# Angel3245/p2pfl

Hardware: AMD Instinct MI355X
Metric: train samples/s (aggregate over peers); wall-clock per FedAvg round in ms_per_step (higher is better)
Workload: dtype bf16; 1 GPU; model=MNIST-CNN (p2pfl CNN: conv5x5 32/64 + FC 3136-2048-10, 6.5M params), Adam 1e-3, global_batch=32, per_peer_round=2700 train + 300 val + 500 test samples, 1 epoch, parallelism=gossip-p2p

## Files before the change

### csrc/cnn.h

```cpp
#pragma once
#include <hip/hip_runtime.h>
#include <stdint.h>

namespace p2cnn {

constexpr int kImg = 28;
constexpr int kC1 = 32;
constexpr int kC2 = 64;
constexpr int kFeat = 3136;
constexpr int kHid = 2048;
constexpr int kCls = 10;
constexpr int kTaps = 25;
constexpr int kXcdSplits = 7;
bool xcd_align();

struct AdamCfg {
  float lr, beta1, beta2, eps, weight_decay;
};

struct Offsets {
  int64_t c1w, c1b, c2w, c2b, l1w, l1b, l2w, l2b;
};

void conv1_fwd(const uint8_t* x, const int64_t* idx, const float* params, Offsets off, uint16_t* p1, uint8_t* am1,
               uint16_t* p1s, int B, hipStream_t s);

void conv2_fwd(const uint16_t* p1, const uint16_t* w2r, const float* params, Offsets off, uint16_t* a1, uint8_t* am2,
               int B, hipStream_t s);

void conv12_fwd(const uint8_t* x, const int64_t* idx, const float* params, Offsets off, const uint16_t* w2r,
                uint16_t* p1, uint8_t* am1, uint16_t* p1s, uint16_t* a1, uint8_t* am2, int B, hipStream_t s);

void gemm_skinny(const uint16_t* A, const uint16_t* Bt, float* slabs, int mrows, int N, int K, int S, hipStream_t s);

void head(const float* slabs, int S, int mrows, const float* params, Offsets off, const int64_t* labels,
          const int64_t* idx, int B, int train, uint16_t* H, uint16_t* dH, float* dlogits, float* stats,
          const uint16_t* w2bf, hipStream_t s);

void fc1_wgrad_adam(const uint16_t* dH, const uint16_t* a1, int mrows, float* params, float* m, float* v,
                    float* gdump, uint16_t* w1bf, uint16_t* w1tbf, Offsets off, const int* adam_t, int t_off,
                    AdamCfg cfg, hipStream_t s);

void route_fc2(const uint16_t* dH, const uint16_t* w1t, const uint8_t* am2, int mrows, int B, uint16_t* dc2m,
               float* gb, const float* dlogits, const uint16_t* H, float* params, float* m, float* v, float* gdump,
               Offsets off, const int* adam_t, int t_off, AdamCfg cfg, bool with_fc2, hipStream_t s);

void route_fc2_rm(const uint16_t* dH, const uint16_t* w1, const uint8_t* am2, int mrows, int B, uint16_t* dc2m,
                  float* gb, const float* dlogits, const uint16_t* H, float* params, float* m, float* v,
                  float* gdump, Offsets off, const int* adam_t, int t_off, AdamCfg cfg, bool with_fc2,
                  float* ws, int* ctr, hipStream_t s);

void conv2_bwd(const uint16_t* dc2m, const uint16_t* p1s, const uint8_t* am1, const uint16_t* w2q, const uint8_t* x,
               const int64_t* idx, float* wslab1, float* wslab2, int B, hipStream_t s);

constexpr int kFc1Tiles = ((kFeat + 127) / 128) * (kHid / 32);
struct Fc1Args {
  const uint16_t* dH;
  const uint16_t* a1;
  int mrows;
  float* params;
  float* m;
  float* v;
  float* gdump;
  uint16_t* w1bf;
  uint16_t* w1tbf;
  Offsets off;
  const int* adam_t;
  int t_off;
  AdamCfg cfg;
};

int conv2_bwd_fc1(const uint16_t* dc2m, const uint16_t* p1s, const uint8_t* am1, const uint16_t* w2q, const uint8_t* x,
                  const int64_t* idx, float* wslab1, float* wslab2, int B, const Fc1Args& f, int n_tiles,
                  hipStream_t s);

void conv_adam(const float* wslab1, const float* wslab2, const float* gb, int B, float* params, float* m, float* v,
               float* gdump, uint16_t* w2r, uint16_t* w2q, Offsets off, const int* adam_t, int t_off, AdamCfg cfg,
               hipStream_t s);

struct FwdNext {
  const uint8_t* x;
  const int64_t* idx;
  uint16_t* p1;
  uint8_t* am1;
  uint16_t* p1s;
  uint16_t* a1;
  uint8_t* am2;
  int B;
  int* sync;
};
void fc1_conv_adam_fwd(const uint16_t* dH, const uint16_t* a1, int mrows, const float* wslab1, const float* wslab2,
                       const float* gb, int B, float* params, float* m, float* v, float* gdump, uint16_t* w1bf,
                       uint16_t* w1tbf, uint16_t* w2r, uint16_t* w2q, Offsets off, const int* adam_t, int t_off,
                       AdamCfg cfg, const float* dlogits, const uint16_t* H, uint16_t* w2bf, const FwdNext& f,
                       hipStream_t s);

void fc1_conv_adam(const uint16_t* dH, const uint16_t* a1, int mrows, const float* wslab1, const float* wslab2,
                   const float* gb, int B, float* params, float* m, float* v, float* gdump, uint16_t* w1bf,
                   uint16_t* w1tbf, uint16_t* w2r, uint16_t* w2q, Offsets off, const int* adam_t, int t_off,
                   AdamCfg cfg, const float* dlogits, const uint16_t* H, uint16_t* w2bf, int first_tile,
                   hipStream_t s);

void pack_shadows(const float* params, Offsets off, uint16_t* w2r, uint16_t* w2q, uint16_t* w1bf, uint16_t* w1tbf,
                  uint16_t* w2bf, hipStream_t s);

constexpr int kP1sPlane = 18 * 16;
constexpr int kP1s = 5 * kC1 * kP1sPlane;
constexpr int kDgTiles = 7;
constexpr int kSlab1 = kC1 * kTaps + kC1;
constexpr int kWgG = 2;
constexpr int kSlab2 = kTaps * kC2 * kC1;
__host__ __device__ inline int wgrad_groups(int B) { return (B + kWgG - 1) / kWgG; }

}
```

### csrc/cnn_bindings.cpp

```cpp
#include <torch/extension.h>
#include <c10/hip/HIPStream.h>
#include <c10/core/DeviceGuard.h>

#include "cnn.h"

namespace {

using p2cnn::AdamCfg;
using p2cnn::Offsets;

hipStream_t stream() { return c10::hip::getCurrentHIPStream().stream(); }

template <typename T>
T* ptr(const torch::Tensor& t, c10::ScalarType st, int64_t min_numel, const char* name, int align = 16) {
  TORCH_CHECK(t.defined() && t.is_cuda(), name, ": expected a GPU tensor");
  TORCH_CHECK(t.scalar_type() == st, name, ": wrong dtype ", t.scalar_type());
  TORCH_CHECK(t.is_contiguous(), name, ": must be contiguous");
  TORCH_CHECK(t.numel() >= min_numel, name, ": needs >= ", min_numel, " elements, got ", t.numel());
  TORCH_CHECK(reinterpret_cast<uintptr_t>(t.data_ptr()) % align == 0, name, ": must be ", align, "-byte aligned");
  return reinterpret_cast<T*>(t.data_ptr());
}
template <typename T>
T* optr(const c10::optional<torch::Tensor>& t, c10::ScalarType st, int64_t min_numel, const char* name,
        int align = 16) {
  if (!t.has_value() || !t->defined()) return nullptr;
  return ptr<T>(*t, st, min_numel, name, align);
}

Offsets offsets(const std::vector<int64_t>& o) {
  TORCH_CHECK(o.size() == 8, "offsets: expected 8 entries");
  for (auto v : o) TORCH_CHECK(v >= 0, "offsets: negative");
  return Offsets{o[0], o[1], o[2], o[3], o[4], o[5], o[6], o[7]};
}

int64_t params_end(const Offsets& o) {
  return std::max({o.c1w + 800, o.c1b + 32, o.c2w + 51200, o.c2b + 64, o.l1w + int64_t(2048) * 3136, o.l1b + 2048,
                   o.l2w + 20480, o.l2b + 10});
}

void check_batch(int B, int mrows) {
  TORCH_CHECK(mrows == 32 || mrows == 64 || mrows == 128, "mrows must be 32, 64 or 128");
  TORCH_CHECK(B >= 1 && B <= mrows, "batch ", B, " exceeds mrows ", mrows);
}

const int64_t* idx_ptr(const c10::optional<torch::Tensor>& idx, int B) {
  return optr<int64_t>(idx, torch::kInt64, B, "idx", 8);
}


void k_conv1_fwd(torch::Tensor x, c10::optional<torch::Tensor> idx, torch::Tensor params, std::vector<int64_t> off,
                 torch::Tensor p1, torch::Tensor am1, c10::optional<torch::Tensor> p1s, int64_t B) {
  const c10::DeviceGuard g(params.device());
  TORCH_CHECK(B >= 1 && B <= (p1s.has_value() && p1s->defined() ? 64 : 128), "bad batch");
  Offsets o = offsets(off);
  TORCH_CHECK(x.numel() % 784 == 0, "x must be [N,1,28,28] uint8");
  if (!idx.has_value()) TORCH_CHECK(x.numel() / 784 >= B, "x has fewer than B rows");
  p2cnn::conv1_fwd(ptr<uint8_t>(x, torch::kUInt8, 784, "x", 1), idx_ptr(idx, B),
                   ptr<float>(params, torch::kFloat32, params_end(o), "params"), o,
                   reinterpret_cast<uint16_t*>(ptr<at::BFloat16>(p1, torch::kBFloat16, B * 196 * 32, "p1")),
                   ptr<uint8_t>(am1, torch::kUInt8, B * 196 * 32, "am1"),
                   reinterpret_cast<uint16_t*>(optr<at::BFloat16>(p1s, torch::kBFloat16, B * p2cnn::kP1s, "p1s")),
                   int(B), stream());
}

void k_conv2_fwd(torch::Tensor p1, torch::Tensor w2r, torch::Tensor params, std::vector<int64_t> off,
                 torch::Tensor a1, torch::Tensor am2, int64_t B, int64_t mrows) {
  const c10::DeviceGuard g(params.device());
  check_batch(int(B), int(mrows));
  Offsets o = offsets(off);
  p2cnn::conv2_fwd(reinterpret_cast<uint16_t*>(ptr<at::BFloat16>(p1, torch::kBFloat16, B * 196 * 32, "p1")),
                   reinterpret_cast<uint16_t*>(ptr<at::BFloat16>(w2r, torch::kBFloat16, 51200, "w2r")),
                   ptr<float>(params, torch::kFloat32, params_end(o), "params"), o,
                   reinterpret_cast<uint16_t*>(ptr<at::BFloat16>(a1, torch::kBFloat16, mrows * 3136, "a1")),
                   ptr<uint8_t>(am2, torch::kUInt8, B * 3136, "am2"), int(B), stream());
}

void k_conv12_fwd(torch::Tensor x, c10::optional<torch::Tensor> idx, torch::Tensor params, std::vector<int64_t> off,
                  torch::Tensor w2r, c10::optional<torch::Tensor> p1, torch::Tensor am1, c10::optional<torch::Tensor> p1s,
                  torch::Tensor a1, torch::Tensor am2, int64_t B, int64_t mrows) {
  const c10::DeviceGuard g(params.device());
  check_batch(int(B), int(mrows));
  TORCH_CHECK(!(p1s.has_value() && p1s->defined()) || B <= 64, "conv12_fwd: training launches hold <= 64 images");
  Offsets o = offsets(off);
  TORCH_CHECK(x.numel() % 784 == 0, "x must be [N,1,28,28] uint8");
  if (!idx.has_value()) TORCH_CHECK(x.numel() / 784 >= B, "x has fewer than B rows");
  p2cnn::conv12_fwd(ptr<uint8_t>(x, torch::kUInt8, 784, "x", 1), idx_ptr(idx, int(B)),
                    ptr<float>(params, torch::kFloat32, params_end(o), "params"), o,
                    reinterpret_cast<uint16_t*>(ptr<at::BFloat16>(w2r, torch::kBFloat16, 51200, "w2r")),
                    reinterpret_cast<uint16_t*>(optr<at::BFloat16>(p1, torch::kBFloat16, B * 196 * 32, "p1")),
                    ptr<uint8_t>(am1, torch::kUInt8, B * 196 * 32, "am1"),
                    reinterpret_cast<uint16_t*>(optr<at::BFloat16>(p1s, torch::kBFloat16, B * p2cnn::kP1s, "p1s")),
                    reinterpret_cast<uint16_t*>(ptr<at::BFloat16>(a1, torch::kBFloat16, mrows * 3136, "a1")),
                    ptr<uint8_t>(am2, torch::kUInt8, B * 3136, "am2"), int(B), stream());
}

void k_gemm_skinny(torch::Tensor A, torch::Tensor Bt, torch::Tensor slabs, int64_t mrows, int64_t N, int64_t K,
                   int64_t S) {
  const c10::DeviceGuard g(A.device());
  TORCH_CHECK(N % 32 == 0 && K % 64 == 0 && S >= 1, "gemm_skinny: N%32, K%64 required");
  TORCH_CHECK(mrows == 32 || mrows == 64 || mrows == 128, "gemm_skinny: mrows must be 32, 64 or 128");
  p2cnn::gemm_skinny(reinterpret_cast<uint16_t*>(ptr<at::BFloat16>(A, torch::kBFloat16, mrows * K, "A")),
                     reinterpret_cast<uint16_t*>(ptr<at::BFloat16>(Bt, torch::kBFloat16, N * K, "Bt")),
                     ptr<float>(slabs, torch::kFloat32, S * mrows * N, "slabs"), int(mrows), int(N), int(K), int(S),
                     stream());
}

void k_head(torch::Tensor slabs, int64_t S, int64_t mrows, torch::Tensor params, std::vector<int64_t> off,
            torch::Tensor labels, c10::optional<torch::Tensor> idx, int64_t B, bool train, torch::Tensor H,
            torch::Tensor dH, torch::Tensor dlogits, torch::Tensor stats, c10::optional<torch::Tensor> w2bf) {
  const c10::DeviceGuard g(params.device());
  check_batch(int(B), int(mrows));
  Offsets o = offsets(off);
  if (!idx.has_value()) TORCH_CHECK(labels.numel() >= B, "labels has fewer than B rows");
  p2cnn::head(ptr<float>(slabs, torch::kFloat32, S * mrows * 2048, "slabs"), int(S), int(mrows),
              ptr<float>(params, torch::kFloat32, params_end(o), "params"), o,
              ptr<int64_t>(labels, torch::kInt64, 1, "labels", 8), idx_ptr(idx, B), int(B), train ? 1 : 0,
              reinterpret_cast<uint16_t*>(ptr<at::BFloat16>(H, torch::kBFloat16, mrows * 2048, "H")),
              reinterpret_cast<uint16_t*>(ptr<at::BFloat16>(dH, torch::kBFloat16, mrows * 2048, "dH")),
              ptr<float>(dlogits, torch::kFloat32, mrows * 10, "dlogits"), ptr<float>(stats, torch::kFloat32, 2, "stats", 4),
              reinterpret_cast<const uint16_t*>(optr<at::BFloat16>(w2bf, torch::kBFloat16, 10 * 2048, "w2bf")),
              stream());
}

AdamCfg cfg(double lr, double b1, double b2, double eps, double wd) {
  return AdamCfg{float(lr), float(b1), float(b2), float(eps), float(wd)};
}

void k_fc1_wgrad_adam(torch::Tensor dH, torch::Tensor a1, int64_t mrows, torch::Tensor params, torch::Tensor m,
                      torch::Tensor v, c10::optional<torch::Tensor> gdump, torch::Tensor w1bf, c10::optional<torch::Tensor> w1tbf,
                      std::vector<int64_t> off, torch::Tensor adam_t, int64_t t_off, double lr, double b1, double b2,
                      double eps, double wd) {
  const c10::DeviceGuard g(params.device());
  TORCH_CHECK(mrows == 32 || mrows == 64, "mrows must be 32 or 64");
  Offsets o = offsets(off);
  const int64_t n = params_end(o);
  p2cnn::fc1_wgrad_adam(reinterpret_cast<uint16_t*>(ptr<at::BFloat16>(dH, torch::kBFloat16, mrows * 2048, "dH")),
                        reinterpret_cast<uint16_t*>(ptr<at::BFloat16>(a1, torch::kBFloat16, mrows * 3136, "a1")),
                        int(mrows), ptr<float>(params, torch::kFloat32, n, "params"),
                        ptr<float>(m, torch::kFloat32, n, "m"), ptr<float>(v, torch::kFloat32, n, "v"),
                        optr<float>(gdump, torch::kFloat32, n, "gdump"),
                        reinterpret_cast<uint16_t*>(ptr<at::BFloat16>(w1bf, torch::kBFloat16, 2048 * 3136, "w1bf")),
                        reinterpret_cast<uint16_t*>(optr<at::BFloat16>(w1tbf, torch::kBFloat16, 2048 * 3136, "w1tbf")),
                        o, ptr<int>(adam_t, torch::kInt32, 1, "adam_t", 4), int(t_off), cfg(lr, b1, b2, eps, wd), stream());
}

void k_route_fc2(torch::Tensor dH, torch::Tensor w1, torch::Tensor am2, int64_t mrows, int64_t B,
                 torch::Tensor dc2m, torch::Tensor gb, torch::Tensor dlogits, torch::Tensor H, torch::Tensor params,
                 torch::Tensor m, torch::Tensor v, c10::optional<torch::Tensor> gdump, std::vector<int64_t> off,
                 torch::Tensor adam_t, int64_t t_off, double lr, double b1, double b2, double eps, double wd,
                 bool with_fc2, bool row_major, c10::optional<torch::Tensor> ws, c10::optional<torch::Tensor> ctr) {
  const c10::DeviceGuard g(dH.device());
  check_batch(int(B), int(mrows));
  TORCH_CHECK(mrows <= 64, "route_fc2: mrows must be 32 or 64");
  TORCH_CHECK(ws.has_value() == ctr.has_value(), "route_fc2: split-K needs both ws and ctr");
  TORCH_CHECK(!ws.has_value() || row_major, "route_fc2: split-K only on the row-major W1 kernel");
  Offsets o = offsets(off);
  const int64_t n = params_end(o);
  const auto dHp = reinterpret_cast<uint16_t*>(ptr<at::BFloat16>(dH, torch::kBFloat16, mrows * 2048, "dH"));
  const auto w1p = reinterpret_cast<uint16_t*>(ptr<at::BFloat16>(w1, torch::kBFloat16, 2048 * 3136, "w1"));
  const auto am2p = ptr<uint8_t>(am2, torch::kUInt8, B * 3136, "am2");
  const auto dc2p = reinterpret_cast<uint16_t*>(ptr<at::BFloat16>(dc2m, torch::kBFloat16, B * 64 * 224, "dc2m"));
  const auto gbp = ptr<float>(gb, torch::kFloat32, B * 3136, "gb");
  const auto dlp = ptr<float>(dlogits, torch::kFloat32, B * 10, "dlogits");
  const auto Hp = reinterpret_cast<uint16_t*>(ptr<at::BFloat16>(H, torch::kBFloat16, B * 2048, "H"));
  float* pp = ptr<float>(params, torch::kFloat32, n, "params");
  float* mp = ptr<float>(m, torch::kFloat32, n, "m");
  float* vp = ptr<float>(v, torch::kFloat32, n, "v");
  float* gd = optr<float>(gdump, torch::kFloat32, n, "gdump");
  const int* tp = ptr<int>(adam_t, torch::kInt32, 1, "adam_t", 4);
  if (row_major) {
    float* wsp = optr<float>(ws, torch::kFloat32, 98 * 2 * mrows * 32, "ws");
    int* cp = optr<int>(ctr, torch::kInt32, 98, "ctr", 4);
    p2cnn::route_fc2_rm(dHp, w1p, am2p, int(mrows), int(B), dc2p, gbp, dlp, Hp, pp, mp, vp, gd, o, tp, int(t_off),
                        cfg(lr, b1, b2, eps, wd), with_fc2, wsp, cp, stream());
  } else {
    p2cnn::route_fc2(dHp, w1p, am2p, int(mrows), int(B), dc2p, gbp, dlp, Hp, pp, mp, vp, gd, o, tp, int(t_off),
                     cfg(lr, b1, b2, eps, wd), with_fc2, stream());
  }
}

int64_t conv2_bwd_impl(torch::Tensor dc2m, torch::Tensor p1s, torch::Tensor am1, torch::Tensor w2q, torch::Tensor x,
                       c10::optional<torch::Tensor> idx, torch::Tensor wslab1, torch::Tensor wslab2, int64_t B,
                       const p2cnn::Fc1Args& fc, int64_t n_tiles) {
  TORCH_CHECK(B >= 1 && B <= 64, "bad batch");
  TORCH_CHECK(x.numel() % 784 == 0, "x must be [N,1,28,28] uint8");
  if (!idx.has_value()) TORCH_CHECK(x.numel() / 784 >= B, "x has fewer than B rows");
  return p2cnn::conv2_bwd_fc1(
      reinterpret_cast<uint16_t*>(ptr<at::BFloat16>(dc2m, torch::kBFloat16, B * 64 * 224, "dc2m")),
      reinterpret_cast<uint16_t*>(ptr<at::BFloat16>(p1s, torch::kBFloat16, B * p2cnn::kP1s, "p1s")),
      ptr<uint8_t>(am1, torch::kUInt8, B * 196 * 32, "am1"),
      reinterpret_cast<uint16_t*>(ptr<at::BFloat16>(w2q, torch::kBFloat16, 51200, "w2q")),
      ptr<uint8_t>(x, torch::kUInt8, 784, "x", 1), idx_ptr(idx, B),
      ptr<float>(wslab1, torch::kFloat32, B * p2cnn::kDgTiles * p2cnn::kSlab1, "wslab1"),
      ptr<float>(wslab2, torch::kFloat32, p2cnn::wgrad_groups(int(B)) * int64_t(p2cnn::kSlab2), "wslab2"), int(B), fc,
      int(n_tiles), stream());
}

void k_conv2_bwd(torch::Tensor dc2m, torch::Tensor p1s, torch::Tensor am1, torch::Tensor w2q, torch::Tensor x,
                 c10::optional<torch::Tensor> idx, torch::Tensor wslab1, torch::Tensor wslab2, int64_t B) {
  const c10::DeviceGuard g(dc2m.device());
  conv2_bwd_impl(dc2m, p1s, am1, w2q, x, idx, wslab1, wslab2, B, p2cnn::Fc1Args{}, 0);
}

int64_t k_conv2_bwd_fc1(torch::Tensor dc2m, torch::Tensor p1s, torch::Tensor am1, torch::Tensor w2q, torch::Tensor x,
                        c10::optional<torch::Tensor> idx, torch::Tensor wslab1, torch::Tensor wslab2, int64_t B,
                        torch::Tensor dH, torch::Tensor a1, int64_t mrows, torch::Tensor params, torch::Tensor m,
                        torch::Tensor v, c10::optional<torch::Tensor> gdump, torch::Tensor w1bf,
                        c10::optional<torch::Tensor> w1tbf, std::vector<int64_t> off, torch::Tensor adam_t,
                        int64_t t_off, double lr, double b1, double b2, double eps, double wd, int64_t n_tiles) {
  const c10::DeviceGuard g(dc2m.device());
  TORCH_CHECK(mrows == 32 || mrows == 64, "conv2_bwd_fc1: mrows must be 32 or 64");
  TORCH_CHECK(n_tiles >= 0 && n_tiles <= p2cnn::kFc1Tiles, "conv2_bwd_fc1: n_tiles ", n_tiles, " outside [0, ",
              p2cnn::kFc1Tiles, "]");
  Offsets o = offsets(off);
  const int64_t n = params_end(o);
  p2cnn::Fc1Args fc{};
  fc.dH = reinterpret_cast<uint16_t*>(ptr<at::BFloat16>(dH, torch::kBFloat16, mrows * 2048, "dH"));
  fc.a1 = reinterpret_cast<uint16_t*>(ptr<at::BFloat16>(a1, torch::kBFloat16, mrows * 3136, "a1"));
  fc.mrows = int(mrows);
  fc.params = ptr<float>(params, torch::kFloat32, n, "params");
  fc.m = ptr<float>(m, torch::kFloat32, n, "m");
  fc.v = ptr<float>(v, torch::kFloat32, n, "v");
  fc.gdump = optr<float>(gdump, torch::kFloat32, n, "gdump");
  fc.w1bf = reinterpret_cast<uint16_t*>(ptr<at::BFloat16>(w1bf, torch::kBFloat16, 2048 * 3136, "w1bf"));
  fc.w1tbf = reinterpret_cast<uint16_t*>(optr<at::BFloat16>(w1tbf, torch::kBFloat16, 2048 * 3136, "w1tbf"));
  fc.off = o;
  fc.adam_t = ptr<int>(adam_t, torch::kInt32, 1, "adam_t", 4);
  fc.t_off = int(t_off);
  fc.cfg = cfg(lr, b1, b2, eps, wd);
  return conv2_bwd_impl(dc2m, p1s, am1, w2q, x, idx, wslab1, wslab2, B, fc, n_tiles);
}

void k_conv_adam(torch::Tensor wslab1, torch::Tensor wslab2, torch::Tensor gb, int64_t B, torch::Tensor params,
                 torch::Tensor m,
                 torch::Tensor v, c10::optional<torch::Tensor> gdump, torch::Tensor w2r, torch::Tensor w2q,
                 std::vector<int64_t> off, torch::Tensor adam_t, int64_t t_off, double lr, double b1, double b2,
                 double eps, double wd) {
  const c10::DeviceGuard g(params.device());
  Offsets o = offsets(off);
  const int64_t n = params_end(o);
  TORCH_CHECK(B >= 1 && B <= 64, "bad batch");
  p2cnn::conv_adam(ptr<float>(wslab1, torch::kFloat32, B * p2cnn::kDgTiles * p2cnn::kSlab1, "wslab1"),
                   ptr<float>(wslab2, torch::kFloat32, p2cnn::wgrad_groups(int(B)) * int64_t(p2cnn::kSlab2), "wslab2"),
                   ptr<float>(gb, torch::kFloat32, B * 3136, "gb"), int(B),
                   ptr<float>(params, torch::kFloat32, n, "params"), ptr<float>(m, torch::kFloat32, n, "m"),
                   ptr<float>(v, torch::kFloat32, n, "v"), optr<float>(gdump, torch::kFloat32, n, "gdump"),
                   reinterpret_cast<uint16_t*>(ptr<at::BFloat16>(w2r, torch::kBFloat16, 51200, "w2r")),
                   reinterpret_cast<uint16_t*>(ptr<at::BFloat16>(w2q, torch::kBFloat16, 51200, "w2q")), o,
                   ptr<int>(adam_t, torch::kInt32, 1, "adam_t", 4), int(t_off), cfg(lr, b1, b2, eps, wd), stream());
}

void k_fc1_conv_adam(torch::Tensor dH, torch::Tensor a1, int64_t mrows, torch::Tensor wslab1, torch::Tensor wslab2,
                     torch::Tensor gb, int64_t B, torch::Tensor params, torch::Tensor m, torch::Tensor v,
                     c10::optional<torch::Tensor> gdump, torch::Tensor w1bf, c10::optional<torch::Tensor> w1tbf, torch::Tensor w2r,
                     torch::Tensor w2q, std::vector<int64_t> off, torch::Tensor adam_t, int64_t t_off, double lr,
                     double b1, double b2, double eps, double wd, c10::optional<torch::Tensor> dlogits,
                     c10::optional<torch::Tensor> H, c10::optional<torch::Tensor> w2bf, int64_t first_tile) {
  const c10::DeviceGuard g(params.device());
  check_batch(int(B), int(mrows));
  TORCH_CHECK(mrows <= 64, "fc1_conv_adam: mrows must be 32 or 64");
  TORCH_CHECK(first_tile >= 0 && first_tile <= p2cnn::kFc1Tiles, "fc1_conv_adam: first_tile ", first_tile,
              " outside [0, ", p2cnn::kFc1Tiles, "]");
  TORCH_CHECK(dlogits.has_value() == H.has_value(), "fc1_conv_adam: pass both dlogits and H or neither");
  Offsets o = offsets(off);
  const int64_t n = params_end(o);
  p2cnn::fc1_conv_adam(
      reinterpret_cast<uint16_t*>(ptr<at::BFloat16>(dH, torch::kBFloat16, mrows * 2048, "dH")),
      reinterpret_cast<uint16_t*>(ptr<at::BFloat16>(a1, torch::kBFloat16, mrows * 3136, "a1")), int(mrows),
      ptr<float>(wslab1, torch::kFloat32, B * p2cnn::kDgTiles * p2cnn::kSlab1, "wslab1"),
      ptr<float>(wslab2, torch::kFloat32, p2cnn::wgrad_groups(int(B)) * int64_t(p2cnn::kSlab2), "wslab2"),
      ptr<float>(gb, torch::kFloat32, B * 3136, "gb"), int(B), ptr<float>(params, torch::kFloat32, n, "params"),
      ptr<float>(m, torch::kFloat32, n, "m"), ptr<float>(v, torch::kFloat32, n, "v"),
      optr<float>(gdump, torch::kFloat32, n, "gdump"),
      reinterpret_cast<uint16_t*>(ptr<at::BFloat16>(w1bf, torch::kBFloat16, 2048 * 3136, "w1bf")),
      reinterpret_cast<uint16_t*>(optr<at::BFloat16>(w1tbf, torch::kBFloat16, 2048 * 3136, "w1tbf")),
      reinterpret_cast<uint16_t*>(ptr<at::BFloat16>(w2r, torch::kBFloat16, 51200, "w2r")),
      reinterpret_cast<uint16_t*>(ptr<at::BFloat16>(w2q, torch::kBFloat16, 51200, "w2q")), o,
      ptr<int>(adam_t, torch::kInt32, 1, "adam_t", 4), int(t_off), cfg(lr, b1, b2, eps, wd),
      optr<float>(dlogits, torch::kFloat32, B * 10, "dlogits"),
      reinterpret_cast<const uint16_t*>(optr<at::BFloat16>(H, torch::kBFloat16, B * 2048, "H")),
      reinterpret_cast<uint16_t*>(optr<at::BFloat16>(w2bf, torch::kBFloat16, 10 * 2048, "w2bf")), int(first_tile),
      stream());
}

void k_fc1_conv_adam_fwd(torch::Tensor dH, torch::Tensor a1, int64_t mrows, torch::Tensor wslab1, torch::Tensor wslab2,
                         torch::Tensor gb, int64_t B, torch::Tensor params, torch::Tensor m, torch::Tensor v,
                         c10::optional<torch::Tensor> gdump, torch::Tensor w1bf, c10::optional<torch::Tensor> w1tbf,
                         torch::Tensor w2r, torch::Tensor w2q, std::vector<int64_t> off, torch::Tensor adam_t,
                         int64_t t_off, double lr, double b1, double b2, double eps, double wd,
                         c10::optional<torch::Tensor> dlogits, c10::optional<torch::Tensor> H,
                         c10::optional<torch::Tensor> w2bf, torch::Tensor x, c10::optional<torch::Tensor> idx,
                         torch::Tensor p1, torch::Tensor am1, torch::Tensor p1s, torch::Tensor a1n, torch::Tensor am2,
                         int64_t Bn, torch::Tensor sync) {
  const c10::DeviceGuard g(params.device());
  check_batch(int(B), int(mrows));
  check_batch(int(Bn), int(mrows));
  TORCH_CHECK(mrows <= 64, "fc1_conv_adam_fwd: mrows must be 32 or 64");
  TORCH_CHECK(dlogits.has_value() == H.has_value(), "fc1_conv_adam_fwd: pass both dlogits and H or neither");
  TORCH_CHECK(x.numel() % 784 == 0, "x must be [N,1,28,28] uint8");
  if (!idx.has_value()) TORCH_CHECK(x.numel() / 784 >= Bn, "x has fewer than Bn rows");
  TORCH_CHECK(a1n.data_ptr() != a1.data_ptr(), "fc1_conv_adam_fwd: the next step's A1 must be the other buffer");
  Offsets o = offsets(off);
  const int64_t n = params_end(o);
  p2cnn::FwdNext f{};
  f.x = ptr<uint8_t>(x, torch::kUInt8, 784, "x", 1);
  f.idx = idx_ptr(idx, int(Bn));
  f.p1 = reinterpret_cast<uint16_t*>(ptr<at::BFloat16>(p1, torch::kBFloat16, Bn * 196 * 32, "p1"));
  f.am1 = ptr<uint8_t>(am1, torch::kUInt8, Bn * 196 * 32, "am1");
  f.p1s = reinterpret_cast<uint16_t*>(ptr<at::BFloat16>(p1s, torch::kBFloat16, Bn * p2cnn::kP1s, "p1s"));
  f.a1 = reinterpret_cast<uint16_t*>(ptr<at::BFloat16>(a1n, torch::kBFloat16, mrows * 3136, "a1n"));
  f.am2 = ptr<uint8_t>(am2, torch::kUInt8, Bn * 3136, "am2");
  f.B = int(Bn);
  f.sync = ptr<int>(sync, torch::kInt32, 4, "sync", 4);
  p2cnn::fc1_conv_adam_fwd(
      reinterpret_cast<uint16_t*>(ptr<at::BFloat16>(dH, torch::kBFloat16, mrows * 2048, "dH")),
      reinterpret_cast<uint16_t*>(ptr<at::BFloat16>(a1, torch::kBFloat16, mrows * 3136, "a1")), int(mrows),
      ptr<float>(wslab1, torch::kFloat32, B * p2cnn::kDgTiles * p2cnn::kSlab1, "wslab1"),
      ptr<float>(wslab2, torch::kFloat32, p2cnn::wgrad_groups(int(B)) * int64_t(p2cnn::kSlab2), "wslab2"),
      ptr<float>(gb, torch::kFloat32, B * 3136, "gb"), int(B), ptr<float>(params, torch::kFloat32, n, "params"),
      ptr<float>(m, torch::kFloat32, n, "m"), ptr<float>(v, torch::kFloat32, n, "v"),
      optr<float>(gdump, torch::kFloat32, n, "gdump"),
      reinterpret_cast<uint16_t*>(ptr<at::BFloat16>(w1bf, torch::kBFloat16, 2048 * 3136, "w1bf")),
      reinterpret_cast<uint16_t*>(optr<at::BFloat16>(w1tbf, torch::kBFloat16, 2048 * 3136, "w1tbf")),
      reinterpret_cast<uint16_t*>(ptr<at::BFloat16>(w2r, torch::kBFloat16, 51200, "w2r")),
      reinterpret_cast<uint16_t*>(ptr<at::BFloat16>(w2q, torch::kBFloat16, 51200, "w2q")), o,
      ptr<int>(adam_t, torch::kInt32, 1, "adam_t", 4), int(t_off), cfg(lr, b1, b2, eps, wd),
      optr<float>(dlogits, torch::kFloat32, B * 10, "dlogits"),
      reinterpret_cast<const uint16_t*>(optr<at::BFloat16>(H, torch::kBFloat16, B * 2048, "H")),
      reinterpret_cast<uint16_t*>(optr<at::BFloat16>(w2bf, torch::kBFloat16, 10 * 2048, "w2bf")), f, stream());
}

void k_pack_shadows(torch::Tensor params, std::vector<int64_t> off, torch::Tensor w2r, torch::Tensor w2q,
                    torch::Tensor w1bf, c10::optional<torch::Tensor> w1tbf, c10::optional<torch::Tensor> w2bf) {
  const c10::DeviceGuard g(params.device());
  Offsets o = offsets(off);
  p2cnn::pack_shadows(ptr<float>(params, torch::kFloat32, params_end(o), "params"), o,
                      reinterpret_cast<uint16_t*>(ptr<at::BFloat16>(w2r, torch::kBFloat16, 51200, "w2r")),
                      reinterpret_cast<uint16_t*>(ptr<at::BFloat16>(w2q, torch::kBFloat16, 51200, "w2q")),
                      reinterpret_cast<uint16_t*>(ptr<at::BFloat16>(w1bf, torch::kBFloat16, 2048 * 3136, "w1bf")),
                      reinterpret_cast<uint16_t*>(optr<at::BFloat16>(w1tbf, torch::kBFloat16, 2048 * 3136, "w1tbf")),
                      reinterpret_cast<uint16_t*>(optr<at::BFloat16>(w2bf, torch::kBFloat16, 10 * 2048, "w2bf")),
                      stream());
}

}

namespace p2cnn {
void init_attributes();
}

void register_cnn(pybind11::module& m) {
  auto c = m.def_submodule("cnn", "fused MNIST-CNN training step kernels");
  c.def("init", &p2cnn::init_attributes, "set kernel attributes (call before HIP graph capture)");
  c.def("conv1_fwd", &k_conv1_fwd);
  c.def("conv2_fwd", &k_conv2_fwd);
  c.def("conv12_fwd", &k_conv12_fwd);
  c.def("gemm_skinny", &k_gemm_skinny);
  c.def("head", &k_head, pybind11::arg("slabs"), pybind11::arg("S"), pybind11::arg("mrows"), pybind11::arg("params"),
        pybind11::arg("off"), pybind11::arg("labels"), pybind11::arg("idx"), pybind11::arg("B"), pybind11::arg("train"),
        pybind11::arg("H"), pybind11::arg("dH"), pybind11::arg("dlogits"), pybind11::arg("stats"),
        pybind11::arg("w2bf") = pybind11::none());
  c.def("route_fc2", &k_route_fc2, pybind11::arg("dH"), pybind11::arg("w1"), pybind11::arg("am2"), pybind11::arg("mrows"), pybind11::arg("B"),
        pybind11::arg("dc2m"), pybind11::arg("gb"), pybind11::arg("dlogits"), pybind11::arg("H"), pybind11::arg("params"), pybind11::arg("m"), pybind11::arg("v"),
        pybind11::arg("gdump"), pybind11::arg("off"), pybind11::arg("adam_t"), pybind11::arg("t_off"), pybind11::arg("lr"), pybind11::arg("b1"),
        pybind11::arg("b2"), pybind11::arg("eps"), pybind11::arg("wd"), pybind11::arg("with_fc2") = true, pybind11::arg("row_major") = false,
        pybind11::arg("ws") = pybind11::none(), pybind11::arg("ctr") = pybind11::none());
  c.def("fc1_wgrad_adam", &k_fc1_wgrad_adam);
  c.def("conv2_bwd", &k_conv2_bwd);
  c.def("conv2_bwd_fc1", &k_conv2_bwd_fc1,
        "conv2_bwd hosting the first n_tiles FC1 weight-gradient + Adam tiles; returns the tiles hosted");
  c.def("conv_adam", &k_conv_adam);
  c.def("fc1_conv_adam", &k_fc1_conv_adam, pybind11::arg("dH"), pybind11::arg("a1"), pybind11::arg("mrows"), pybind11::arg("wslab1"),
        pybind11::arg("wslab2"), pybind11::arg("gb"), pybind11::arg("B"), pybind11::arg("params"), pybind11::arg("m"), pybind11::arg("v"), pybind11::arg("gdump"),
        pybind11::arg("w1bf"), pybind11::arg("w1tbf"), pybind11::arg("w2r"), pybind11::arg("w2q"), pybind11::arg("off"), pybind11::arg("adam_t"),
        pybind11::arg("t_off"), pybind11::arg("lr"), pybind11::arg("b1"), pybind11::arg("b2"), pybind11::arg("eps"), pybind11::arg("wd"),
        pybind11::arg("dlogits") = pybind11::none(), pybind11::arg("H") = pybind11::none(),
        pybind11::arg("w2bf") = pybind11::none(), pybind11::arg("first_tile") = 0);
  c.def("fc1_conv_adam_fwd", &k_fc1_conv_adam_fwd);
  c.def("pack_shadows", &k_pack_shadows, pybind11::arg("params"), pybind11::arg("off"), pybind11::arg("w2r"),
        pybind11::arg("w2q"), pybind11::arg("w1bf"), pybind11::arg("w1tbf"), pybind11::arg("w2bf") = pybind11::none());
  c.def("wgrad_groups", [](int64_t B) { return int64_t(p2cnn::wgrad_groups(int(B))); },
        "conv2 weight-gradient partial slabs (of 51200 floats) written for a batch of B");
}
```

### csrc/cnn_bwd.hip

```cpp
#include <cstdlib>

#include "cnn.h"
#include "cnn_fwd_dev.h"
#include "common.h"

namespace p2cnn {
using namespace p2;

typedef __bf16 bf16x8_t __attribute__((ext_vector_type(8)));
typedef short s16x4 __attribute__((ext_vector_type(4)));
P2_DEVICE f32x16 mfma32b(uint4 a, uint4 b, f32x16 c) {
  return __builtin_amdgcn_mfma_f32_32x32x16_bf16(__builtin_bit_cast(bf16x8_t, a), __builtin_bit_cast(bf16x8_t, b), c,
                                                  0, 0, 0);
}
P2_DEVICE int acc_row_b(int i, int h) { return (i & 3) + 8 * (i >> 2) + 4 * h; }
P2_DEVICE uint4 pack8(const uint16_t (&v)[8]) {
  uint4 q;
  q.x = uint32_t(v[0]) | (uint32_t(v[1]) << 16);
  q.y = uint32_t(v[2]) | (uint32_t(v[3]) << 16);
  q.z = uint32_t(v[4]) | (uint32_t(v[5]) << 16);
  q.w = uint32_t(v[6]) | (uint32_t(v[7]) << 16);
  return q;
}

struct AdamScal {
  float step_size, inv_sqrt_bc2;
};
P2_DEVICE AdamScal adam_scal(const AdamCfg& c, const int* t, int t_off) {
  const float tt = float(*t + t_off);
  AdamScal s;
  s.step_size = c.lr / (1.f - powf(c.beta1, tt));
  s.inv_sqrt_bc2 = 1.f / sqrtf(1.f - powf(c.beta2, tt));
  return s;
}
P2_DEVICE float adam_dir(float mv, float vv, float c, float eps) {
  return mv * __builtin_amdgcn_rcpf(fmaf(__builtin_amdgcn_sqrtf(vv), c, eps));
}
P2_DEVICE void adam_regs(float& pv, float& mv, float& vv, float g, const AdamCfg& c, const AdamScal& s) {
  if (c.weight_decay != 0.f) g = fmaf(c.weight_decay, pv, g);
  mv = fmaf(c.beta1, mv, (1.f - c.beta1) * g);
  vv = fmaf(c.beta2, vv, (1.f - c.beta2) * g * g);
  pv -= s.step_size * adam_dir(mv, vv, s.inv_sqrt_bc2, c.eps);
}
P2_DEVICE float adam_apply(float* __restrict__ p, float* __restrict__ m, float* __restrict__ v, int64_t e, float g,
                           const AdamCfg& c, const AdamScal& s) {
  float pv = p[e];
  if (c.weight_decay != 0.f) g = fmaf(c.weight_decay, pv, g);
  const float mv = fmaf(c.beta1, m[e], (1.f - c.beta1) * g);
  const float vv = fmaf(c.beta2, v[e], (1.f - c.beta2) * g * g);
  pv -= s.step_size * adam_dir(mv, vv, s.inv_sqrt_bc2, c.eps);
  p[e] = pv;
  m[e] = mv;
  v[e] = vv;
  return pv;
}

constexpr int kRouteBlocks = kFeat / 32;
constexpr int kFc2Blocks = (kCls * kHid + kCls + 511) / 512;

template <int TPB>
P2_DEVICE void fc2_role(int blk, const float* __restrict__ dlogits, const uint16_t* __restrict__ H, int B,
                        float* __restrict__ p, float* __restrict__ m, float* __restrict__ v,
                        float* __restrict__ gdump, const Offsets& off, const int* __restrict__ adam_t, int t_off,
                        const AdamCfg& cfg, uint16_t* __restrict__ w2bf = nullptr) {
  const int e = blk * TPB + threadIdx.x;
  const int nW = kCls * kHid;
  if (e >= nW + kCls) return;
  const int64_t pi = e < nW ? off.l2w + e : off.l2b + (e - nW);
  float pv = p[pi], mv = m[pi], vv = v[pi];
  float g = 0.f;
  if (e < nW) {
    const int c = e / kHid, k = e % kHid;
    for (int b0 = 0; b0 < B; b0 += 8) {
      float t[8];
#pragma unroll
      for (int u = 0; u < 8; ++u)
        t[u] = b0 + u < B ? dlogits[(b0 + u) * kCls + c] * bf16_to_f32(H[size_t(b0 + u) * kHid + k]) : 0.f;
#pragma unroll
      for (int u = 0; u < 8; ++u) g += t[u];
    }
  } else {
    const int c = e - nW;
    for (int b = 0; b < B; ++b) g += dlogits[b * kCls + c];
  }
  if (gdump) gdump[pi] = g;
  const AdamScal s = adam_scal(cfg, adam_t, t_off);
  adam_regs(pv, mv, vv, g, cfg, s);
  p[pi] = pv;
  m[pi] = mv;
  v[pi] = vv;
  if (w2bf && e < nW) w2bf[e] = f32_to_bf16(pv);
}

template <int MT>
__global__ __launch_bounds__(512) void route_fc2_kernel(const uint16_t* __restrict__ dH,
                                                        const uint16_t* __restrict__ w1t,
                                                        const uint8_t* __restrict__ am2, int B,
                                                        uint16_t* __restrict__ dc2m, float* __restrict__ gb,
                                                        const float* __restrict__ dlogits,
                                                        const uint16_t* __restrict__ H, float* __restrict__ p,
                                                        float* __restrict__ m, float* __restrict__ v,
                                                        float* __restrict__ gdump, Offsets off,
                                                        const int* __restrict__ adam_t, int t_off, AdamCfg cfg) {
  const int bid = blockIdx.x;
  if (bid >= kRouteBlocks) {
    fc2_role<512>(bid - kRouteBlocks, dlogits, H, B, p, m, v, gdump, off, adam_t, t_off, cfg);
    return;
  }
  __shared__ float red[8 * MT * 1024];
  const int tid = threadIdx.x, wave = tid >> 6, lane = tid & 63, r = lane & 31, h = lane >> 5;
  const int n0 = bid * 32;
  constexpr int K = kHid, NG = K / 64;
  uint8_t acode[2 * MT];
#pragma unroll
  for (int q = 0; q < 2 * MT; ++q) {
    const int e = tid + 512 * q;
    const int b = (e >> 10) * 32 + acc_row_b((e >> 6) & 15, (e & 63) >> 5);
    acode[q] = b < B ? am2[size_t(b) * kFeat + n0 + (e & 31)] : uint8_t(4);
  }
  f32x16 acc[MT];
#pragma unroll
  for (int mt = 0; mt < MT; ++mt) acc[mt] = f32x16{};
  const uint16_t* brow = w1t + size_t(n0 + r) * K + 32 * h;
  constexpr int NGW = NG / 8;
  uint4 bq[NGW][4], aq[NGW][MT][4];
#pragma unroll
  for (int gi = 0; gi < NGW; ++gi) {
    const int k0 = (wave + 8 * gi) * 64;
#pragma unroll
    for (int q = 0; q < 4; ++q) bq[gi][q] = ld_nt16(brow + k0 + q * 8);
#pragma unroll
    for (int mt = 0; mt < MT; ++mt)
#pragma unroll
      for (int q = 0; q < 4; ++q)
        aq[gi][mt][q] = reinterpret_cast<const uint4*>(dH + size_t(mt * 32 + r) * K + 32 * h + k0)[q];
  }
  __builtin_amdgcn_sched_barrier(0);
#pragma unroll
  for (int gi = 0; gi < NGW; ++gi)
#pragma unroll
    for (int q = 0; q < 4; ++q)
#pragma unroll
      for (int mt = 0; mt < MT; ++mt) acc[mt] = mfma32b(aq[gi][mt][q], bq[gi][q], acc[mt]);
#pragma unroll
  for (int mt = 0; mt < MT; ++mt)
#pragma unroll
    for (int i = 0; i < 16; ++i) red[((wave * MT + mt) * 16 + i) * 64 + lane] = acc[mt][i];
  __syncthreads();
#pragma unroll
  for (int q = 0; q < 2 * MT; ++q) {
    const int e = tid + 512 * q;
    float g = 0.f;
#pragma unroll
    for (int w = 0; w < 8; ++w) g += red[w * MT * 1024 + e];
    const int mt = e >> 10, i = (e >> 6) & 15, ln = e & 63;
    const int b = mt * 32 + acc_row_b(i, ln >> 5), feat = n0 + (ln & 31);
    if (b >= B) continue;
    const uint8_t a = acode[q];
    const int oc = feat / 49, pp = feat % 49, py = pp / 7, px = pp % 7;
    gb[size_t(b) * kFeat + feat] = a < 4 ? g : 0.f;
    const uint16_t gv = f32_to_bf16(g);
    uint16_t* row = dc2m + (size_t(b) * kC2 + oc) * 224 + (2 * py) * 16 + 2 * px;
    const uint32_t top = (a == 0 ? gv : 0u) | (uint32_t(a == 1 ? gv : 0u) << 16);
    const uint32_t bot = (a == 2 ? gv : 0u) | (uint32_t(a == 3 ? gv : 0u) << 16);
    *reinterpret_cast<uint32_t*>(row) = top;
    *reinterpret_cast<uint32_t*>(row + 16) = bot;
  }
}

constexpr int kRouteRmLds = kHid * 64;

P2_DEVICE int xcd_local(int orig, int nwg) {
  const int xcd = orig % 8, q = nwg / 8, r = nwg % 8;
  return (xcd < r ? xcd * (q + 1) : r * (q + 1) + (xcd - r) * q) + orig / 8;
}

P2_DEVICE void st_sc1f(float* p, float v) {
  const auto rs = __builtin_amdgcn_make_buffer_rsrc(p, 0, 4, 0x00020000);
  __builtin_amdgcn_raw_buffer_store_b32(__float_as_uint(v), rs, 0, 0, 16);
}
P2_DEVICE float ld_sc1f(const float* p) {
  const auto rs = __builtin_amdgcn_make_buffer_rsrc(const_cast<float*>(p), 0, 4, 0x00020000);
  return __uint_as_float(__builtin_amdgcn_raw_buffer_load_b32(rs, 0, 0, 16));
}

template <int MT, int KS>
__global__ __launch_bounds__(512) void route_rm_kernel(const uint16_t* __restrict__ dH,
                                                       const uint16_t* __restrict__ w1,
                                                       const uint8_t* __restrict__ am2, int B,
                                                       uint16_t* __restrict__ dc2m, float* __restrict__ gb,
                                                       const float* __restrict__ dlogits,
                                                       const uint16_t* __restrict__ H, float* __restrict__ p,
                                                       float* __restrict__ m, float* __restrict__ v,
                                                       float* __restrict__ gdump, Offsets off,
                                                       const int* __restrict__ adam_t, int t_off, AdamCfg cfg,
                                                       float* __restrict__ ws, int* __restrict__ ctr, int xa) {
  constexpr int NB = kRouteBlocks * KS;
  const int nbl = xa ? 8 * xa : NB;
  if (int(blockIdx.x) >= nbl) {
    fc2_role<512>(blockIdx.x - nbl, dlogits, H, B, p, m, v, gdump, off, adam_t, t_off, cfg);
    return;
  }
  int bid;
  if (xa) {
    const int x = blockIdx.x & 7, r = blockIdx.x >> 3;
    bid = x * xa + r;
    if (bid >= NB) return;
  } else {
    bid = xcd_local(blockIdx.x, NB);
  }
  const int tile = bid / KS, split = bid % KS;
  extern __shared__ __attribute__((aligned(16))) char smem[];
  static_assert(8 * MT * 1024 * 4 <= kRouteRmLds / KS, "reduction buffer must fit the tile");
  float* red = reinterpret_cast<float*>(smem);
  const int tid = threadIdx.x, wave = tid >> 6, lane = tid & 63, r = lane & 31, h = lane >> 5;
  const int n0 = tile * 32;
  constexpr int K = kHid, NG = K / 64, NGW = NG / 8 / KS;
  const int gbase = split * (NG / KS);
  uint8_t acode[2 * MT];
#pragma unroll
  for (int q = 0; q < 2 * MT; ++q) {
    const int e = tid + 512 * q;
    const int b = (e >> 10) * 32 + acc_row_b((e >> 6) & 15, (e & 63) >> 5);
    acode[q] = b < B ? am2[size_t(b) * kFeat + n0 + (e & 31)] : uint8_t(4);
  }
#pragma unroll
  for (int gi = 0; gi < NGW; ++gi) {
    const int kl = (wave + 8 * gi) * 64, k0 = gbase * 64 + kl;
#pragma unroll
    for (int c = 0; c < 4; ++c) {
      const int row = k0 + 16 * c + (lane >> 2);
      __builtin_amdgcn_global_load_lds(
          (const __attribute__((address_space(1))) void*)(w1 + size_t(row) * kFeat + n0 + (lane & 3) * 8),
          (__attribute__((address_space(3))) void*)(smem + (kl + 16 * c) * 64), 16, 0, 0);
    }
  }
  uint4 aq[NGW][MT][4];
#pragma unroll
  for (int gi = 0; gi < NGW; ++gi) {
    const int k0 = (gbase + wave + 8 * gi) * 64;
#pragma unroll
    for (int mt = 0; mt < MT; ++mt)
#pragma unroll
      for (int q = 0; q < 4; ++q)
        aq[gi][mt][q] = reinterpret_cast<const uint4*>(dH + size_t(mt * 32 + r) * K + 32 * h + k0)[q];
  }
  asm volatile("s_waitcnt vmcnt(0)" ::: "memory");
  __syncthreads();
  f32x16 acc[MT];
#pragma unroll
  for (int mt = 0; mt < MT; ++mt) acc[mt] = f32x16{};
  const int g = lane >> 4, qq = (lane >> 2) & 3, col = 16 * (g & 1) + 4 * (lane & 3);
#pragma unroll
  for (int gi = 0; gi < NGW; ++gi) {
    const int kl = (wave + 8 * gi) * 64;
#pragma unroll
    for (int q = 0; q < 4; ++q) {
      uint4 bq;
#pragma unroll
      for (int t = 0; t < 2; ++t) {
        const int row = kl + 32 * (g >> 1) + 8 * q + 4 * t + qq;
        const s16x4 w = __builtin_amdgcn_ds_read_tr16_b64_v4i16(
            (__attribute__((address_space(3))) s16x4*)(smem + row * 64 + col * 2));
        const uint2 u = __builtin_bit_cast(uint2, w);
        if (t == 0) {
          bq.x = u.x;
          bq.y = u.y;
        } else {
          bq.z = u.x;
          bq.w = u.y;
        }
      }
#pragma unroll
      for (int mt = 0; mt < MT; ++mt) acc[mt] = mfma32b(aq[gi][mt][q], bq, acc[mt]);
    }
  }
  __syncthreads();
#pragma unroll
  for (int mt = 0; mt < MT; ++mt)
#pragma unroll
    for (int i = 0; i < 16; ++i) red[((wave * MT + mt) * 16 + i) * 64 + lane] = acc[mt][i];
  __syncthreads();
  float part[2 * MT];
#pragma unroll
  for (int q = 0; q < 2 * MT; ++q) {
    const int e = tid + 512 * q;
    float gsum = 0.f;
#pragma unroll
    for (int w = 0; w < 8; ++w) gsum += red[w * MT * 1024 + e];
    part[q] = gsum;
  }
  if (KS > 1) {
    float* slab = ws + size_t(tile) * KS * (MT * 1024);
#pragma unroll
    for (int q = 0; q < 2 * MT; ++q) st_sc1f(slab + split * (MT * 1024) + tid + 512 * q, part[q]);
    asm volatile("s_waitcnt vmcnt(0)" ::: "memory");
    __syncthreads();
    int* flag = reinterpret_cast<int*>(smem);
    if (tid == 0) {
      const int old = __hip_atomic_fetch_add(ctr + tile, 1, __ATOMIC_RELAXED, __HIP_MEMORY_SCOPE_AGENT);
      flag[0] = old == KS - 1;
      if (old == KS - 1) __hip_atomic_store(ctr + tile, 0, __ATOMIC_RELAXED, __HIP_MEMORY_SCOPE_AGENT);
    }
    __syncthreads();
    if (!flag[0]) return;
#pragma unroll
    for (int q = 0; q < 2 * MT; ++q) {
      float t = 0.f;
#pragma unroll
      for (int s2 = 0; s2 < KS; ++s2) t += s2 == split ? part[q] : ld_sc1f(slab + s2 * (MT * 1024) + tid + 512 * q);
      part[q] = t;
    }
  }
#pragma unroll
  for (int q = 0; q < 2 * MT; ++q) {
    const int e = tid + 512 * q;
    const float gsum = part[q];
    const int mt = e >> 10, i = (e >> 6) & 15, ln = e & 63;
    const int b = mt * 32 + acc_row_b(i, ln >> 5), feat = n0 + (ln & 31);
    if (b >= B) continue;
    const uint8_t a = acode[q];
    const int oc = feat / 49, pp = feat % 49, py = pp / 7, px = pp % 7;
    gb[size_t(b) * kFeat + feat] = a < 4 ? gsum : 0.f;
    const uint16_t gv = f32_to_bf16(gsum);
    uint16_t* row = dc2m + (size_t(b) * kC2 + oc) * 224 + (2 * py) * 16 + 2 * px;
    const uint32_t top = (a == 0 ? gv : 0u) | (uint32_t(a == 1 ? gv : 0u) << 16);
    const uint32_t bot = (a == 2 ? gv : 0u) | (uint32_t(a == 3 ? gv : 0u) << 16);
    *reinterpret_cast<uint32_t*>(row) = top;
    *reinterpret_cast<uint32_t*>(row + 16) = bot;
  }
}

void route_fc2_rm(const uint16_t* dH, const uint16_t* w1, const uint8_t* am2, int mrows, int B, uint16_t* dc2m,
                  float* gb, const float* dlogits, const uint16_t* H, float* params, float* m, float* v,
                  float* gdump, Offsets off, const int* adam_t, int t_off, AdamCfg cfg, bool with_fc2,
                  float* ws, int* ctr, hipStream_t s) {
  const int ks = (ws && ctr) ? 2 : 1;
  const int xa = (ks == 1 && xcd_align()) ? kRouteBlocks / kXcdSplits : 0;
  static_assert(kRouteBlocks % kXcdSplits == 0 && kXcdSplits <= 8, "routing tiles split evenly over the aligned XCDs");
  const dim3 grid((xa ? 8 * xa : kRouteBlocks * ks) + (with_fc2 ? kFc2Blocks : 0));
  const int lds = kRouteRmLds / ks;
#define P2_ROUTE(MT, KS)                                                                                            \
  hipLaunchKernelGGL((route_rm_kernel<MT, KS>), grid, dim3(512), lds, s, dH, w1, am2, B, dc2m, gb, dlogits, H, params, \
                     m, v, gdump, off, adam_t, t_off, cfg, ws, ctr, xa)
  if (mrows == 32) {
    if (ks == 2) P2_ROUTE(1, 2); else P2_ROUTE(1, 1);
  } else {
    if (ks == 2) P2_ROUTE(2, 2); else P2_ROUTE(2, 1);
  }
#undef P2_ROUTE
}

void route_fc2(const uint16_t* dH, const uint16_t* w1t, const uint8_t* am2, int mrows, int B, uint16_t* dc2m,
               float* gb, const float* dlogits, const uint16_t* H, float* params, float* m, float* v, float* gdump,
               Offsets off, const int* adam_t, int t_off, AdamCfg cfg, bool with_fc2, hipStream_t s) {
  const dim3 grid(kRouteBlocks + (with_fc2 ? kFc2Blocks : 0));
  if (mrows == 32)
    hipLaunchKernelGGL(route_fc2_kernel<1>, grid, dim3(512), 0, s, dH, w1t, am2, B, dc2m, gb, dlogits, H, params, m,
                       v, gdump, off, adam_t, t_off, cfg);
  else
    hipLaunchKernelGGL(route_fc2_kernel<2>, grid, dim3(512), 0, s, dH, w1t, am2, B, dc2m, gb, dlogits, H, params, m,
                       v, gdump, off, adam_t, t_off, cfg);
}

template <int MR>
struct Fc1Lds {
  static constexpr int AP = 144;
  static constexpr int GP = 132;
  static constexpr int kStage = MR * (32 + AP) * 2;
  static constexpr int kGrad = 32 * GP * 4;
  static constexpr int kMain = kStage > kGrad ? kStage : kGrad;
  static constexpr int kBytes = kMain + 128 * 40 * 2;
};

template <int MR>
P2_DEVICE void fc1_wgrad_adam_body(int bx, int by, const uint16_t* __restrict__ dH, const uint16_t* __restrict__ a1,
                                   float* __restrict__ p, float* __restrict__ m, float* __restrict__ v,
                                   float* __restrict__ gdump, uint16_t* __restrict__ w1bf,
                                   uint16_t* __restrict__ w1tbf, const Offsets& off,
                                   const int* __restrict__ adam_t, int t_off, const AdamCfg& cfg, char* smem) {
  constexpr int AP = Fc1Lds<MR>::AP;
  constexpr int GP = Fc1Lds<MR>::GP;
  uint16_t(*tr)[40] = reinterpret_cast<uint16_t(*)[40]>(smem + Fc1Lds<MR>::kMain);
  uint16_t* sdh = reinterpret_cast<uint16_t*>(smem);
  uint16_t* sa1 = sdh + MR * 32;
  float(*gt)[GP] = reinterpret_cast<float(*)[GP]>(smem);
  const int tid = threadIdx.x, wave = tid >> 6, lane = tid & 63, r = lane & 31, h = lane >> 5;
  const int n0 = by * 32;
  const int kb = bx * 128;
  const int nl = tid >> 3, kq = (tid & 7) * 4;
  float* pw = p + off.l1w;
  float* mw = m + off.l1w;
  float* vw = v + off.l1w;
  float4 pr[4], mr[4], vr[4];
#pragma unroll
  for (int j = 0; j < 4; ++j) {
    const int k = kb + kq + 32 * j;
    if (k < kFeat) {
      const int64_t e = int64_t(n0 + nl) * kFeat + k;
      pr[j] = *reinterpret_cast<const float4*>(pw + e);
      mr[j] = *reinterpret_cast<const float4*>(mw + e);
      vr[j] = *reinterpret_cast<const float4*>(vw + e);
    }
  }
  for (int i = tid; i < MR * 4; i += 256) {
    const int b = i >> 2, q = i & 3;
    *reinterpret_cast<uint4*>(sdh + b * 32 + q * 8) = reinterpret_cast<const uint4*>(dH + size_t(b) * kHid + n0)[q];
  }
  for (int i = tid; i < MR * 16; i += 256) {
    const int b = i >> 4, q = i & 15;
    const int k = kb + q * 8;
    uint4 u = make_uint4(0, 0, 0, 0);
    if (k < kFeat) u = reinterpret_cast<const uint4*>(a1 + size_t(b) * kFeat + k)[0];
    *reinterpret_cast<uint4*>(sa1 + b * AP + q * 8) = u;
  }
  __syncthreads();
  const AdamScal s = adam_scal(cfg, adam_t, t_off);
  if (bx == 0 && wave == 0 && lane < 32) {
    const int n = n0 + lane;
    float g = 0.f;
    for (int b = 0; b < MR; ++b) g += bf16_to_f32(sdh[b * 32 + lane]);
    if (gdump) gdump[off.l1b + n] = g;
    adam_apply(p, m, v, off.l1b + n, g, cfg, s);
  }
  const int g4 = lane >> 4, qq = (lane >> 2) & 3, c16 = 16 * (g4 & 1) + 4 * (lane & 3), hh = g4 >> 1;
  f32x16 acc = {};
#pragma unroll
  for (int st = 0; st < MR / 16; ++st) {
    uint4 a, bq;
#pragma unroll
    for (int t = 0; t < 2; ++t) {
      const int row = (MR / 2) * hh + 8 * st + 4 * t + qq;
      const uint2 ua = __builtin_bit_cast(uint2, __builtin_amdgcn_ds_read_tr16_b64_v4i16(
          (__attribute__((address_space(3))) s16x4*)(sdh + row * 32 + c16)));
      const uint2 ub = __builtin_bit_cast(uint2, __builtin_amdgcn_ds_read_tr16_b64_v4i16(
          (__attribute__((address_space(3))) s16x4*)(sa1 + row * AP + wave * 32 + c16)));
      if (t == 0) {
        a.x = ua.x, a.y = ua.y, bq.x = ub.x, bq.y = ub.y;
      } else {
        a.z = ua.x, a.w = ua.y, bq.z = ub.x, bq.w = ub.y;
      }
    }
    acc = mfma32b(a, bq, acc);
  }
  __syncthreads();
#pragma unroll
  for (int i = 0; i < 16; ++i) gt[acc_row_b(i, h)][wave * 32 + r] = acc[i];
  __syncthreads();
#pragma unroll
  for (int j = 0; j < 4; ++j) {
    const int kl = kq + 32 * j, k = kb + kl;
    if (k >= kFeat) continue;
    const float4 g = *reinterpret_cast<const float4*>(&gt[nl][kl]);
    const int64_t e = int64_t(n0 + nl) * kFeat + k;
    if (gdump) *reinterpret_cast<float4*>(gdump + off.l1w + e) = g;
    adam_regs(pr[j].x, mr[j].x, vr[j].x, g.x, cfg, s);
    adam_regs(pr[j].y, mr[j].y, vr[j].y, g.y, cfg, s);
    adam_regs(pr[j].z, mr[j].z, vr[j].z, g.z, cfg, s);
    adam_regs(pr[j].w, mr[j].w, vr[j].w, g.w, cfg, s);
    *reinterpret_cast<float4*>(pw + e) = pr[j];
    *reinterpret_cast<float4*>(mw + e) = mr[j];
    *reinterpret_cast<float4*>(vw + e) = vr[j];
    const uint16_t b0 = f32_to_bf16(pr[j].x), b1 = f32_to_bf16(pr[j].y), b2 = f32_to_bf16(pr[j].z),
                   b3 = f32_to_bf16(pr[j].w);
    uint2 o;
    o.x = uint32_t(b0) | (uint32_t(b1) << 16);
    o.y = uint32_t(b2) | (uint32_t(b3) << 16);
    *reinterpret_cast<uint2*>(w1bf + e) = o;
    if (!w1tbf) continue;
    tr[kl][nl] = b0;
    tr[kl + 1][nl] = b1;
    tr[kl + 2][nl] = b2;
    tr[kl + 3][nl] = b3;
  }
  if (!w1tbf) return;
  __syncthreads();
  for (int j = tid; j < 128 * 4; j += 256) {
    const int kl = j >> 2, q = j & 3;
    const int k = kb + kl;
    if (k < kFeat)
      *reinterpret_cast<uint4*>(w1tbf + size_t(k) * kHid + n0 + q * 8) = *reinterpret_cast<const uint4*>(&tr[kl][q * 8]);
  }
}

template <int MR>
__global__ __launch_bounds__(256) void fc1_wgrad_adam_kernel(const uint16_t* __restrict__ dH, const uint16_t* __restrict__ a1,
                                                             float* __restrict__ p, float* __restrict__ m,
                                                             float* __restrict__ v, float* __restrict__ gdump,
                                                             uint16_t* __restrict__ w1bf, uint16_t* __restrict__ w1tbf,
                                                             Offsets off, const int* __restrict__ adam_t, int t_off,
                                                             AdamCfg cfg) {
  __shared__ __attribute__((aligned(16))) char smem[Fc1Lds<MR>::kBytes];
  fc1_wgrad_adam_body<MR>(blockIdx.x, blockIdx.y, dH, a1, p, m, v, gdump, w1bf, w1tbf, off, adam_t, t_off, cfg, smem);
}

void fc1_wgrad_adam(const uint16_t* dH, const uint16_t* a1, int mrows, float* params, float* m, float* v,
                    float* gdump, uint16_t* w1bf, uint16_t* w1tbf, Offsets off, const int* adam_t, int t_off,
                    AdamCfg cfg, hipStream_t s) {
  const dim3 grid((kFeat + 127) / 128, kHid / 32);
  if (mrows == 32)
    hipLaunchKernelGGL(fc1_wgrad_adam_kernel<32>, grid, dim3(256), 0, s, dH, a1, params, m, v, gdump, w1bf, w1tbf,
                       off, adam_t, t_off, cfg);
  else
    hipLaunchKernelGGL(fc1_wgrad_adam_kernel<64>, grid, dim3(256), 0, s, dH, a1, params, m, v, gdump, w1bf, w1tbf,
                       off, adam_t, t_off, cfg);
}

constexpr int kOCP = 72;

P2_DEVICE void conv2_wgrad_role(int t, int g, const uint16_t* __restrict__ dc2m, const uint16_t* __restrict__ p1s,
                                float* __restrict__ wslab, int B) {
  const int lane = threadIdx.x & 63, r = lane & 31, h = lane >> 5;
  const int ky = t / 5, kx = t % 5;
  const int b0 = g * kWgG, nb = min(kWgG, B - b0);
  auto load = [&](int c, uint4 (&A0)[7], uint4 (&A1)[7], uint4 (&Bv)[7]) {
    const int b = b0 + (c >> 1), row0 = (c & 1) * 7;
    const uint16_t* a = dc2m + (size_t(b) * kC2 + r) * 224 + 8 * h;
    const uint16_t* bb = p1s + ((size_t(b) * 5 + kx) * kC1 + r) * kP1sPlane + ky * 16 + 8 * h;
#pragma unroll
    for (int j = 0; j < 7; ++j) {
      const int ks = row0 + j;
      A0[j] = *reinterpret_cast<const uint4*>(a + ks * 16);
      A1[j] = *reinterpret_cast<const uint4*>(a + 32 * 224 + ks * 16);
      Bv[j] = *reinterpret_cast<const uint4*>(bb + ks * 16);
    }
  };
  f32x16 acc0 = {}, acc1 = {};
  uint4 xa0[7], xa1[7], xb[7], ya0[7], ya1[7], yb[7];
  const int nch = 2 * nb;
  load(0, xa0, xa1, xb);
#pragma unroll
  for (int c = 0; c < 2 * kWgG; c += 2) {
    if (c < nch) {
      if (c + 1 < nch) load(c + 1, ya0, ya1, yb);
      __builtin_amdgcn_sched_barrier(0);
#pragma unroll
      for (int j = 0; j < 7; ++j) {
        acc0 = mfma32b(xa0[j], xb[j], acc0);
        acc1 = mfma32b(xa1[j], xb[j], acc1);
      }
      __builtin_amdgcn_sched_barrier(0);
    }
    if (c + 1 < nch) {
      if (c + 2 < nch) load(c + 2, xa0, xa1, xb);
      __builtin_amdgcn_sched_barrier(0);
#pragma unroll
      for (int j = 0; j < 7; ++j) {
        acc0 = mfma32b(ya0[j], yb[j], acc0);
        acc1 = mfma32b(ya1[j], yb[j], acc1);
      }
      __builtin_amdgcn_sched_barrier(0);
    }
  }
  float* out = wslab + (size_t(g) * kTaps + t) * kC2 * kC1 + r;
#pragma unroll
  for (int i = 0; i < 16; ++i) {
    const int oc = acc_row_b(i, h);
    out[oc * kC1] = acc0[i];
    out[(oc + 32) * kC1] = acc1[i];
  }
}

constexpr int kWgA = kWgG * kC2 * 224 * 2;
constexpr int kWgB = kWgG * kC1 * kP1sPlane * 2;
static_assert(kWgA + kWgB <= 143424, "wgrad staging must fit the launch's LDS");

P2_DEVICE void glds_copy(const uint16_t* src, char* dst, int bytes, int wave, int lane) {
  for (int c = wave; c * 1024 < bytes; c += 4)
    __builtin_amdgcn_global_load_lds((const __attribute__((address_space(1))) void*)(src + c * 512 + lane * 8),
                                     (__attribute__((address_space(3))) void*)(dst + c * 1024), 16, 0, 0);
}

P2_DEVICE int wg_swz(int row) { return (row >> 2) & 3; }

template <int CPR>
P2_DEVICE void glds_copy_swz(const uint16_t* src, char* dst, int bytes, int wave, int lane) {
  static_assert(CPR % 4 == 0, "the swizzle permutes chunk groups of 4 inside a row");
  for (int c = wave; c * 1024 < bytes; c += 4) {
    const int q = c * 64 + lane, rho = q / CPR, j = q - rho * CPR;
    const int sq = rho * CPR + (j ^ wg_swz(rho));
    __builtin_amdgcn_global_load_lds((const __attribute__((address_space(1))) void*)(src + sq * 8),
                                     (__attribute__((address_space(3))) void*)(dst + c * 1024), 16, 0, 0);
  }
}

P2_DEVICE void conv2_wgrad_block(int g, int kx, const uint16_t* __restrict__ dc2m, const uint16_t* __restrict__ p1s,
                                 float* __restrict__ wslab, int B, char* smem) {
  const int tid = threadIdx.x, wave = tid >> 6, lane = tid & 63, r = lane & 31, h = lane >> 5;
  const int b0 = g * kWgG, nb = min(kWgG, B - b0);
  const uint16_t* sa = reinterpret_cast<const uint16_t*>(smem);
  const uint16_t* sb = reinterpret_cast<const uint16_t*>(smem + kWgA);
  static_assert(224 % 32 == 0 && kP1sPlane % 32 == 0, "whole 16-B chunk groups per row");
  glds_copy_swz<224 / 8>(dc2m + size_t(b0) * kC2 * 224, smem, nb * kC2 * 224 * 2, wave, lane);
  for (int i = 0; i < nb; ++i)
    glds_copy_swz<kP1sPlane / 8>(p1s + (size_t(b0 + i) * 5 + kx) * kC1 * kP1sPlane,
                                 smem + kWgA + i * (kC1 * kP1sPlane * 2), kC1 * kP1sPlane * 2, wave, lane);
  asm volatile("s_waitcnt vmcnt(0)" ::: "memory");
  __syncthreads();
  const int t = h ^ wg_swz(r);
  for (int ky = wave; ky < 5; ky += 4) {
    f32x16 acc0 = {}, acc1 = {};
    for (int i = 0; i < nb; ++i) {
      const uint16_t* a = sa + (i * kC2 + r) * 224;
      const uint16_t* bb = sb + (i * kC1 + r) * kP1sPlane;
#pragma unroll
      for (int ks = 0; ks < 14; ++ks) {
        const int ca = (2 * ks) ^ t, cb = (2 * (ky + ks)) ^ t;
        const uint4 a0 = *reinterpret_cast<const uint4*>(a + 8 * ca);
        const uint4 a1 = *reinterpret_cast<const uint4*>(a + 32 * 224 + 8 * ca);
        const uint4 bq = *reinterpret_cast<const uint4*>(bb + 8 * cb);
        acc0 = mfma32b(a0, bq, acc0);
        acc1 = mfma32b(a1, bq, acc1);
      }
    }
    float* out = wslab + (size_t(g) * kTaps + ky * 5 + kx) * kC2 * kC1 + r;
#pragma unroll
    for (int i = 0; i < 16; ++i) {
      const int oc = acc_row_b(i, h);
      out[oc * kC1] = acc0[i];
      out[(oc + 32) * kC1] = acc1[i];
    }
  }
}

constexpr int kW2qRow = kTaps * kC2 + 8;
constexpr int kDgW = kC1 * kW2qRow * 2;
constexpr int kDgWinRows = 14;
constexpr int kDgWin = kDgWinRows * 18 * kOCP * 2;
constexpr int kDgXs = 32 * 33 * 4;
constexpr int kDgLds = kDgW + kDgWin + kDgXs;

template <bool STREAM_W>
P2_DEVICE void conv2_dgrad_block(int grp, int b, const uint16_t* __restrict__ dc2m, const uint8_t* __restrict__ am1,
                                 const uint16_t* __restrict__ w2q, const uint8_t* __restrict__ xds,
                                 const int64_t* __restrict__ idx, float* __restrict__ wslab1, char* smem) {
  uint16_t* sw = reinterpret_cast<uint16_t*>(smem);
  uint16_t* win = reinterpret_cast<uint16_t*>(smem + kDgW);
  float(*xs)[33] = reinterpret_cast<float(*)[33]>(smem + kDgW + kDgWin);
  const int tid = threadIdx.x, wave = tid >> 6, lane = tid & 63, r = lane & 31, h = lane >> 5;
  const int tile = grp * 4 + wave;
  const bool active = tile < kDgTiles;
  const int ylo = grp ? (4 * 32) / 14 : 0;
  const int m = tile * 32 + r, mc = m < 196 ? m : 195;
  const int y = mc / 14, x = mc % 14;
  if (!STREAM_W) {
#pragma unroll 4
    for (int k = 0; k < 32; ++k) {
      const int id = wave * 32 + k, ic = id >> 2, q = id & 3;
      if (lane < 50)
        __builtin_amdgcn_global_load_lds(
            (const __attribute__((address_space(1))) void*)(w2q + ic * (kTaps * kC2) + q * 400 + lane * 8),
            (__attribute__((address_space(3))) void*)(sw + ic * kW2qRow + q * 400), 16, 0, 0);
    }
  }
  uint4 wu0[4], wu1[4];
#pragma unroll
  for (int it = 0; it < 4; ++it) {
    const int i = tid + 256 * it;
    const int wr = i >> 6, pr = (i >> 1) & 31, c = i & 1, yd = ylo + wr - 2;
    const int ydc = yd < 0 ? 0 : (yd > 13 ? 13 : yd);
    const uint16_t* src = dc2m + (size_t(b) * kC2 + 2 * pr) * 224 + ydc * 16 + c * 8;
    wu0[it] = *reinterpret_cast<const uint4*>(src);
    wu1[it] = *reinterpret_cast<const uint4*>(src + 224);
  }
  uint8_t acode[16];
#pragma unroll
  for (int i = 0; i < 16; ++i) {
    const int pos = tile * 32 + acc_row_b(i, h);
    acode[i] = (active && pos < 196) ? am1[(size_t(b) * 196 + pos) * kC1 + r] : uint8_t(4);
  }
  const int64_t row = idx ? idx[b] : b;
  const uint8_t* xsrc = xds + row * (kImg * kImg);
  const uint4 z4 = make_uint4(0, 0, 0, 0);
  for (int i = tid; i < kDgWin / 16; i += 256) reinterpret_cast<uint4*>(win)[i] = z4;
  for (int i = tid; i < 32 * 32; i += 256) {
    const int yy = i >> 5, xx = i & 31, sy = yy - 2, sx = xx - 2;
    float v = 0.f;
    if (sy >= 0 && sy < kImg && sx >= 0 && sx < kImg) v = float(xsrc[sy * kImg + sx]) * (1.f / 255.f);
    xs[yy][xx] = v;
  }
  __syncthreads();
#pragma unroll
  for (int it = 0; it < 4; ++it) {
    const int i = tid + 256 * it;
    const int wr = i >> 6, pr = (i >> 1) & 31, c = i & 1, yd = ylo + wr - 2;
    if (i >= kDgWinRows * 64 || yd < 0 || yd > 13) continue;
    const uint16_t* e0 = reinterpret_cast<const uint16_t*>(&wu0[it]);
    const uint16_t* e1 = reinterpret_cast<const uint16_t*>(&wu1[it]);
    uint16_t* dst = win + (wr * 18 + c * 8 + 2) * kOCP + 2 * pr;
#pragma unroll
    for (int j = 0; j < 8; ++j) *reinterpret_cast<uint32_t*>(dst + j * kOCP) = uint32_t(e0[j]) | (uint32_t(e1[j]) << 16);
  }
  __syncthreads();
  if (!active) return;
  const uint16_t* abase = win + ((y - ylo) * 18 + x) * kOCP + 8 * h;
  f32x16 acc = {};
  if (STREAM_W) {
    const uint16_t* brow = w2q + r * (kTaps * kC2) + 8 * h;
    uint4 bx[10], by[10];
#pragma unroll
    for (int j = 0; j < 10; ++j) bx[j] = *reinterpret_cast<const uint4*>(brow + 16 * j);
#pragma unroll
    for (int c = 0; c < 10; c += 2) {
      if (c + 1 < 10) {
#pragma unroll
        for (int j = 0; j < 10; ++j) by[j] = *reinterpret_cast<const uint4*>(brow + 16 * ((c + 1) * 10 + j));
      }
#pragma unroll
      for (int j = 0; j < 10; ++j) {
        const int s2 = c * 10 + j, t = s2 >> 2, ky = t / 5, kx = t % 5, oc0 = (s2 & 3) * 16;
        const uint4 a = *reinterpret_cast<const uint4*>(abase + ((4 - ky) * 18 + (4 - kx)) * kOCP + oc0);
        acc = mfma32b(a, bx[j], acc);
      }
      if (c + 2 < 10) {
#pragma unroll
        for (int j = 0; j < 10; ++j) bx[j] = *reinterpret_cast<const uint4*>(brow + 16 * ((c + 2) * 10 + j));
      }
#pragma unroll
      for (int j = 0; j < 10; ++j) {
        const int s2 = (c + 1) * 10 + j, t = s2 >> 2, ky = t / 5, kx = t % 5, oc0 = (s2 & 3) * 16;
        const uint4 a = *reinterpret_cast<const uint4*>(abase + ((4 - ky) * 18 + (4 - kx)) * kOCP + oc0);
        acc = mfma32b(a, by[j], acc);
      }
    }
  } else {
    const uint16_t* bbase = sw + r * kW2qRow + 8 * h;
#pragma unroll 4
    for (int s = 0; s < 100; ++s) {
      const int t = s >> 2, ky = t / 5, kx = t % 5, oc0 = (s & 3) * 16;
      const uint4 a = *reinterpret_cast<const uint4*>(abase + ((4 - ky) * 18 + (4 - kx)) * kOCP + oc0);
      const uint4 bq = *reinterpret_cast<const uint4*>(bbase + t * kC2 + oc0);
      acc = mfma32b(a, bq, acc);
    }
  }
  float wg[kTaps];
#pragma unroll
  for (int t = 0; t < kTaps; ++t) wg[t] = 0.f;
  float bs = 0.f;
#pragma unroll
  for (int i = 0; i < 16; ++i) {
    const int pos = tile * 32 + acc_row_b(i, h);
    const uint8_t a = acode[i];
    if (pos < 196 && a < 4) {
      const int yy = 2 * (pos / 14) + (a >> 1), xx = 2 * (pos % 14) + (a & 1);
      const float gv = acc[i];
      bs += gv;
#pragma unroll
      for (int ky = 0; ky < 5; ++ky)
#pragma unroll
        for (int kx = 0; kx < 5; ++kx) wg[ky * 5 + kx] = fmaf(gv, xs[yy + ky][xx + kx], wg[ky * 5 + kx]);
    }
  }
#pragma unroll
  for (int t = 0; t < kTaps; ++t) wg[t] += __shfl_xor(wg[t], 32, 64);
  bs += __shfl_xor(bs, 32, 64);
  if (h == 0) {
    float* o = wslab1 + (size_t(b) * kDgTiles + tile) * kSlab1;
#pragma unroll
    for (int t = 0; t < kTaps; ++t) o[r * kTaps + t] = wg[t];
    o[kC1 * kTaps + r] = bs;
  }
}

P2_DEVICE void conv2_bwd_roles(int j, int nconv, const uint16_t* __restrict__ dc2m, const uint16_t* __restrict__ p1s,
                               const uint8_t* __restrict__ am1, const uint16_t* __restrict__ w2q,
                               const uint8_t* __restrict__ xds, const int64_t* __restrict__ idx,
                               float* __restrict__ wslab1, float* __restrict__ wslab2, int B, int wg_blocks,
                               int stream_w, int wg_first, char* smem) {
  const int nd = 2 * B;
  if (wg_first) j = j < nconv - nd ? j + nd : j - (nconv - nd);
  if (j < nd) {
    if (stream_w)
      conv2_dgrad_block<true>(j & 1, j >> 1, dc2m, am1, w2q, xds, idx, wslab1, smem);
    else
      conv2_dgrad_block<false>(j & 1, j >> 1, dc2m, am1, w2q, xds, idx, wslab1, smem);
  } else if (wg_blocks) {
    const int k = j - nd;
    conv2_wgrad_block(k / 5, k % 5, dc2m, p1s, wslab2, B, smem);
  } else {
    const int k = (j - nd) * 4 + (threadIdx.x >> 6);
    if (k < kTaps * wgrad_groups(B)) conv2_wgrad_role(k % kTaps, k / kTaps, dc2m, p1s, wslab2, B);
  }
}

__global__ __launch_bounds__(256) void conv2_bwd_kernel(const uint16_t* __restrict__ dc2m,
                                                        const uint16_t* __restrict__ p1s,
                                                        const uint8_t* __restrict__ am1,
                                                        const uint16_t* __restrict__ w2q,
                                                        const uint8_t* __restrict__ xds,
                                                        const int64_t* __restrict__ idx, float* __restrict__ wslab1,
                                                        float* __restrict__ wslab2, int B, int first_block,
                                                        int wg_blocks, int stream_w, int wg_first) {
  extern __shared__ __attribute__((aligned(16))) char smem[];
  conv2_bwd_roles(blockIdx.x + first_block, gridDim.x, dc2m, p1s, am1, w2q, xds, idx, wslab1, wslab2, B, wg_blocks,
                  stream_w, wg_first, smem);
}

template <int MR>
__global__ __launch_bounds__(256) void conv2_bwd_fc1_kernel(
    const uint16_t* __restrict__ dc2m, const uint16_t* __restrict__ p1s, const uint8_t* __restrict__ am1,
    const uint16_t* __restrict__ w2q, const uint8_t* __restrict__ xds, const int64_t* __restrict__ idx,
    float* __restrict__ wslab1, float* __restrict__ wslab2, int B, int nconv, int wg_blocks, int stream_w,
    int wg_first, Fc1Args f) {
  static_assert(Fc1Lds<MR>::kBytes <= kDgLds, "the launch's dynamic LDS serves the FC1 role too");
  extern __shared__ __attribute__((aligned(16))) char smem[];
  constexpr int kBx = (kFeat + 127) / 128;
  const int j = blockIdx.x;
  if (j < nconv) {
    conv2_bwd_roles(j, nconv, dc2m, p1s, am1, w2q, xds, idx, wslab1, wslab2, B, wg_blocks, stream_w, wg_first, smem);
    return;
  }
  const int t = j - nconv;
  fc1_wgrad_adam_body<MR>(t % kBx, t / kBx, f.dH, f.a1, f.params, f.m, f.v, f.gdump, f.w1bf, f.w1tbf, f.off, f.adam_t,
                          f.t_off, f.cfg, smem);
}

int conv2_bwd_fc1(const uint16_t* dc2m, const uint16_t* p1s, const uint8_t* am1, const uint16_t* w2q, const uint8_t* x,
                  const int64_t* idx, float* wslab1, float* wslab2, int B, const Fc1Args& f, int n_tiles,
                  hipStream_t s) {
  static const int roles = [] {
    const char* e = getenv("P2CNN_CONV2BWD_ROLES");
    return e ? atoi(e) : 3;
  }();
  static const int wg_blocks = [] {
    const char* e = getenv("P2CNN_CONV2_WG_BLOCKS");
    return e ? atoi(e) : 1;
  }();
  static const int stream_w = [] {
    const char* e = getenv("P2CNN_DGRAD_STREAM_W");
    return e ? atoi(e) : 0;
  }();
  static const int wg_first = [] {
    const char* e = getenv("P2CNN_CONV2BWD_WG_FIRST");
    return e ? atoi(e) : 0;
  }();
  const int nd = 2 * B, nw = wg_blocks ? 5 * wgrad_groups(B) : (kTaps * wgrad_groups(B) + 3) / 4;
  const int first = roles == 2 ? nd : 0;
  const int blocks = roles == 1 ? nd : roles == 2 ? nw : nd + nw;
  const int na = roles == 3 ? n_tiles : 0;
  if (na == 0)
    hipLaunchKernelGGL(conv2_bwd_kernel, dim3(blocks), dim3(256), kDgLds, s, dc2m, p1s, am1, w2q, x, idx, wslab1,
                       wslab2, B, first, wg_blocks, stream_w, roles == 3 ? wg_first : 0);
  else if (f.mrows == 32)
    hipLaunchKernelGGL(conv2_bwd_fc1_kernel<32>, dim3(blocks + na), dim3(256), kDgLds, s, dc2m, p1s, am1, w2q, x, idx,
                       wslab1, wslab2, B, blocks, wg_blocks, stream_w, wg_first, f);
  else
    hipLaunchKernelGGL(conv2_bwd_fc1_kernel<64>, dim3(blocks + na), dim3(256), kDgLds, s, dc2m, p1s, am1, w2q, x, idx,
                       wslab1, wslab2, B, blocks, wg_blocks, stream_w, wg_first, f);
  return na;
}

void conv2_bwd(const uint16_t* dc2m, const uint16_t* p1s, const uint8_t* am1, const uint16_t* w2q, const uint8_t* x,
               const int64_t* idx, float* wslab1, float* wslab2, int B, hipStream_t s) {
  conv2_bwd_fc1(dc2m, p1s, am1, w2q, x, idx, wslab1, wslab2, B, Fc1Args{}, 0, s);
}

constexpr int kC1Blocks = kSlab1 / 16;

constexpr int kConvAdamLds = (kTaps * (kC1 + 1) + 256) * 4;

template <bool WT>
P2_DEVICE void st_p(float* p, float v) {
  if constexpr (WT)
    __hip_atomic_store(p, v, __ATOMIC_RELAXED, __HIP_MEMORY_SCOPE_AGENT);
  else
    *p = v;
}
template <bool WT>
P2_DEVICE void st_h(uint16_t* p, uint16_t v) {
  if constexpr (WT)
    __hip_atomic_store(p, v, __ATOMIC_RELAXED, __HIP_MEMORY_SCOPE_AGENT);
  else
    *p = v;
}

template <bool WT = false>
P2_DEVICE void conv_adam_body(int blk, const float* __restrict__ ws1, const float* __restrict__ ws2,
                              const float* __restrict__ gb, int B, float* __restrict__ p, float* __restrict__ m,
                              float* __restrict__ v, float* __restrict__ gdump, uint16_t* __restrict__ w2r,
                              uint16_t* __restrict__ w2q, const Offsets& off, const int* __restrict__ adam_t, int t_off,
                              const AdamCfg& cfg, char* smem) {
  float(*g2)[kC1 + 1] = reinterpret_cast<float(*)[kC1 + 1]>(smem);
  float* red = reinterpret_cast<float*>(smem + kTaps * (kC1 + 1) * 4);
  const int tid = threadIdx.x;
  const AdamScal sc = adam_scal(cfg, adam_t, t_off);
  if (blk < kC2) {
    const int oc = blk, ng = wgrad_groups(B);
    float pr[4], mr[4], vr[4];
#pragma unroll
    for (int u = 0; u < 4; ++u) {
      const int j = tid + 256 * u;
      const int64_t e = off.c2w + int64_t(oc) * kC1 * kTaps + (j < kC1 * kTaps ? j : 0);
      pr[u] = p[e];
      mr[u] = m[e];
      vr[u] = v[e];
    }
    float pb = 0.f, mb = 0.f, vb = 0.f;
    if (tid == 0) {
      pb = p[off.c2b + oc];
      mb = m[off.c2b + oc];
      vb = v[off.c2b + oc];
    }
    float acc[4] = {0.f, 0.f, 0.f, 0.f};
    for (int g0 = 0; g0 < ng; g0 += 8) {
      float t[4][8];
#pragma unroll
      for (int u = 0; u < 4; ++u)
#pragma unroll
        for (int k = 0; k < 8; ++k) {
          const int j = tid + 256 * u, t_ = j >> 5, ic = j & 31, gg = g0 + k;
          t[u][k] = (j < kTaps * kC1 && gg < ng) ? ws2[((size_t(gg) * kTaps + t_) * kC2 + oc) * kC1 + ic] : 0.f;
        }
#pragma unroll
      for (int u = 0; u < 4; ++u)
#pragma unroll
        for (int k = 0; k < 8; ++k) acc[u] += t[u][k];
    }
#pragma unroll
    for (int u = 0; u < 4; ++u) {
      const int j = tid + 256 * u;
      if (j < kTaps * kC1) g2[j >> 5][j & 31] = acc[u];
    }
    float bs = 0.f;
    for (int e0 = 0; e0 < B * 49; e0 += 256 * 8) {
      float t[8];
#pragma unroll
      for (int u = 0; u < 8; ++u) {
        const int e = e0 + tid + 256 * u;
        t[u] = e < B * 49 ? gb[size_t(e / 49) * kFeat + oc * 49 + e % 49] : 0.f;
      }
#pragma unroll
      for (int u = 0; u < 8; ++u) bs += t[u];
    }
    red[tid] = bs;
    __syncthreads();
    for (int w = 128; w > 0; w >>= 1) {
      if (tid < w) red[tid] += red[tid + w];
      __syncthreads();
    }
#pragma unroll
    for (int u = 0; u < 4; ++u) {
      const int j = tid + 256 * u;
      if (j >= kC1 * kTaps) break;
      const int ic = j / kTaps, t = j % kTaps;
      const float g = g2[t][ic];
      const int64_t e = off.c2w + int64_t(oc) * kC1 * kTaps + j;
      if (gdump) gdump[e] = g;
      adam_regs(pr[u], mr[u], vr[u], g, cfg, sc);
      st_p<WT>(p + e, pr[u]);
      m[e] = mr[u];
      v[e] = vr[u];
      const uint16_t hb = f32_to_bf16(pr[u]);
      st_h<WT>(w2r + (oc * kTaps + t) * kC1 + ic, hb);
      w2q[(ic * kTaps + t) * kC2 + oc] = hb;
    }
    if (tid == 0) {
      if (gdump) gdump[off.c2b + oc] = red[0];
      adam_regs(pb, mb, vb, red[0], cfg, sc);
      st_p<WT>(p + off.c2b + oc, pb);
      m[off.c2b + oc] = mb;
      v[off.c2b + oc] = vb;
    }
  } else {
    const int j = (blk - kC2) * 16 + (tid & 15), q = tid >> 4;
    const int rows = B * kDgTiles;
    const int64_t e = j < kC1 * kTaps ? off.c1w + j : off.c1b + (j - kC1 * kTaps);
    float pe = 0.f, me = 0.f, ve = 0.f;
    if (q == 0) {
      pe = p[e];
      me = m[e];
      ve = v[e];
    }
    float s = 0.f;
    for (int r0 = q; r0 < rows; r0 += 16 * 8) {
      float t[8];
#pragma unroll
      for (int u = 0; u < 8; ++u) {
        const int rw = r0 + 16 * u;
        t[u] = rw < rows ? ws1[size_t(rw) * kSlab1 + j] : 0.f;
      }
#pragma unroll
      for (int u = 0; u < 8; ++u) s += t[u];
    }
    red[tid] = s;
    __syncthreads();
    if (q == 0) {
      float g = 0.f;
#pragma unroll
      for (int k = 0; k < 16; ++k) g += red[k * 16 + tid];
      if (gdump) gdump[e] = g;
      adam_regs(pe, me, ve, g, cfg, sc);
      st_p<WT>(p + e, pe);
      m[e] = me;
      v[e] = ve;
    }
  }
}

__global__ __launch_bounds__(256) void conv_adam_kernel(const float* __restrict__ ws1, const float* __restrict__ ws2,
                                                        const float* __restrict__ gb, int B, float* __restrict__ p,
                                                        float* __restrict__ m, float* __restrict__ v,
                                                        float* __restrict__ gdump, uint16_t* __restrict__ w2r,
                                                        uint16_t* __restrict__ w2q, Offsets off,
                                                        const int* __restrict__ adam_t, int t_off, AdamCfg cfg) {
  __shared__ __attribute__((aligned(16))) char smem[kConvAdamLds];
  conv_adam_body(blockIdx.x, ws1, ws2, gb, B, p, m, v, gdump, w2r, w2q, off, adam_t, t_off, cfg, smem);
}

constexpr int kFc2Blocks256 = (kCls * kHid + kCls + 255) / 256;

template <int MR>
__global__ __launch_bounds__(256) void fc1_conv_adam_kernel(
    const uint16_t* __restrict__ dH, const uint16_t* __restrict__ a1, const float* __restrict__ ws1,
    const float* __restrict__ ws2, const float* __restrict__ gb, int B, float* __restrict__ p, float* __restrict__ m,
    float* __restrict__ v, float* __restrict__ gdump, uint16_t* __restrict__ w1bf, uint16_t* __restrict__ w1tbf,
    uint16_t* __restrict__ w2r, uint16_t* __restrict__ w2q, Offsets off, const int* __restrict__ adam_t, int t_off,
    AdamCfg cfg, const float* __restrict__ dlogits, const uint16_t* __restrict__ H, int nf2,
    uint16_t* __restrict__ w2bf, int f0) {
  constexpr int kLds = Fc1Lds<MR>::kBytes > kConvAdamLds ? Fc1Lds<MR>::kBytes : kConvAdamLds;
  __shared__ __attribute__((aligned(16))) char smem[kLds];
  constexpr int kCA = kC2 + kC1Blocks, kBx = (kFeat + 127) / 128;
  int j = blockIdx.x;
  if (j < nf2) {
    fc2_role<256>(j, dlogits, H, B, p, m, v, gdump, off, adam_t, t_off, cfg, w2bf);
    return;
  }
  j -= nf2;
  if (j < kCA) {
    conv_adam_body(j, ws1, ws2, gb, B, p, m, v, gdump, w2r, w2q, off, adam_t, t_off, cfg, smem);
    return;
  }
  const int f = j - kCA + f0;
  fc1_wgrad_adam_body<MR>(f % kBx, f / kBx, dH, a1, p, m, v, gdump, w1bf, w1tbf, off, adam_t, t_off, cfg, smem);
}

void fc1_conv_adam(const uint16_t* dH, const uint16_t* a1, int mrows, const float* wslab1, const float* wslab2,
                   const float* gb, int B, float* params, float* m, float* v, float* gdump, uint16_t* w1bf,
                   uint16_t* w1tbf, uint16_t* w2r, uint16_t* w2q, Offsets off, const int* adam_t, int t_off,
                   AdamCfg cfg, const float* dlogits, const uint16_t* H, uint16_t* w2bf, int first_tile,
                   hipStream_t s) {
  const int nf2 = dlogits ? kFc2Blocks256 : 0;
  const dim3 grid(nf2 + kC2 + kC1Blocks + kFc1Tiles - first_tile);
  if (mrows == 32)
    hipLaunchKernelGGL(fc1_conv_adam_kernel<32>, grid, dim3(256), 0, s, dH, a1, wslab1, wslab2, gb, B, params, m, v,
                       gdump, w1bf, w1tbf, w2r, w2q, off, adam_t, t_off, cfg, dlogits, H, nf2, w2bf, first_tile);
  else
    hipLaunchKernelGGL(fc1_conv_adam_kernel<64>, grid, dim3(256), 0, s, dH, a1, wslab1, wslab2, gb, B, params, m, v,
                       gdump, w1bf, w1tbf, w2r, w2q, off, adam_t, t_off, cfg, dlogits, H, nf2, w2bf, first_tile);
}

P2_DEVICE void wait_tickets(int* ctr, int target, int* stall) {
  if (threadIdx.x == 0) {
    int it = 0;
    while (__hip_atomic_load(ctr, __ATOMIC_RELAXED, __HIP_MEMORY_SCOPE_AGENT) < target) {
      if (++it > (1 << 22)) {
        __hip_atomic_store(stall, 1, __ATOMIC_RELAXED, __HIP_MEMORY_SCOPE_AGENT);
        break;
      }
      __builtin_amdgcn_s_sleep(2);
    }
  }
  __syncthreads();
}
P2_DEVICE void put_ticket(int* ctr) {
  asm volatile("s_waitcnt vmcnt(0)" ::: "memory");
  __syncthreads();
  if (threadIdx.x == 0) __hip_atomic_fetch_add(ctr, 1, __ATOMIC_RELAXED, __HIP_MEMORY_SCOPE_AGENT);
}

template <int MR>
__global__ __launch_bounds__(256) void fc1_conv_adam_fwd_kernel(
    const uint16_t* __restrict__ dH, const uint16_t* __restrict__ a1, const float* __restrict__ ws1,
    const float* __restrict__ ws2, const float* __restrict__ gb, int B, float* __restrict__ p, float* __restrict__ m,
    float* __restrict__ v, float* __restrict__ gdump, uint16_t* __restrict__ w1bf, uint16_t* __restrict__ w1tbf,
    uint16_t* __restrict__ w2r, uint16_t* __restrict__ w2q, Offsets off, const int* __restrict__ adam_t, int t_off,
    AdamCfg cfg, const float* __restrict__ dlogits, const uint16_t* __restrict__ H, int nf2,
    uint16_t* __restrict__ w2bf, FwdNext f) {
  constexpr int kA = Fc1Lds<MR>::kBytes > kConvAdamLds ? Fc1Lds<MR>::kBytes : kConvAdamLds;
  constexpr int kB = int(sizeof(Conv1Smem)) > 4 * 32 * 33 * 4 ? int(sizeof(Conv1Smem)) : 4 * 32 * 33 * 4;
  __shared__ __attribute__((aligned(16))) char smem[kA > kB ? kA : kB];
  constexpr int kCA = kC2 + kC1Blocks, kBx = (kFeat + 127) / 128;
  const int n1 = 7 * f.B, n2 = (14 * f.B + 3) / 4;
  int j = blockIdx.x;
  if (j < nf2) {
    fc2_role<256>(j, dlogits, H, B, p, m, v, gdump, off, adam_t, t_off, cfg, w2bf);
    return;
  }
  j -= nf2;
  if (j < kCA) {
    conv_adam_body<true>(j, ws1, ws2, gb, B, p, m, v, gdump, w2r, w2q, off, adam_t, t_off, cfg, smem);
    put_ticket(f.sync);
    return;
  }
  j -= kCA;
  constexpr int nfc1 = kBx * (kHid / 32);
  if (j < nfc1) {
    fc1_wgrad_adam_body<MR>(j % kBx, j / kBx, dH, a1, p, m, v, gdump, w1bf, w1tbf, off, adam_t, t_off, cfg, smem);
    return;
  }
  j -= nfc1;
  if (j < n1) {
    wait_tickets(f.sync, kCA, f.sync + 3);
    conv1_body<true>(j % 7, j / 7, f.x, f.idx, p + off.c1w, p + off.c1b, f.p1, f.am1, f.p1s,
                     *reinterpret_cast<Conv1Smem*>(smem));
    put_ticket(f.sync + 1);
    return;
  }
  j -= n1;
  if (j < n2) {
    wait_tickets(f.sync + 1, n1, f.sync + 3);
    const int wave = threadIdx.x >> 6, item = j * 4 + wave;
    float(*sout)[33] = reinterpret_cast<float(*)[33]>(smem + wave * (32 * 33 * 4));
    conv2_body<true>(item < 14 * f.B, item % 7, (item / 7) & 1, item / 14, threadIdx.x & 63, f.p1, w2r, p + off.c2b,
                     f.a1, f.am2, sout);
    __syncthreads();
    if (threadIdx.x == 0 &&
        __hip_atomic_fetch_add(f.sync + 2, 1, __ATOMIC_RELAXED, __HIP_MEMORY_SCOPE_AGENT) == n2 - 1) {
      __hip_atomic_store(f.sync, 0, __ATOMIC_RELAXED, __HIP_MEMORY_SCOPE_AGENT);
      __hip_atomic_store(f.sync + 1, 0, __ATOMIC_RELAXED, __HIP_MEMORY_SCOPE_AGENT);
      __hip_atomic_store(f.sync + 2, 0, __ATOMIC_RELAXED, __HIP_MEMORY_SCOPE_AGENT);
    }
  }
}

void fc1_conv_adam_fwd(const uint16_t* dH, const uint16_t* a1, int mrows, const float* wslab1, const float* wslab2,
                       const float* gb, int B, float* params, float* m, float* v, float* gdump, uint16_t* w1bf,
                       uint16_t* w1tbf, uint16_t* w2r, uint16_t* w2q, Offsets off, const int* adam_t, int t_off,
                       AdamCfg cfg, const float* dlogits, const uint16_t* H, uint16_t* w2bf, const FwdNext& f,
                       hipStream_t s) {
  const int nf2 = dlogits ? kFc2Blocks256 : 0;
  const int n1 = 7 * f.B, n2 = (14 * f.B + 3) / 4;
  const dim3 grid(nf2 + kC2 + kC1Blocks + n1 + n2 + ((kFeat + 127) / 128) * (kHid / 32));
  if (mrows == 32)
    hipLaunchKernelGGL(fc1_conv_adam_fwd_kernel<32>, grid, dim3(256), 0, s, dH, a1, wslab1, wslab2, gb, B, params, m,
                       v, gdump, w1bf, w1tbf, w2r, w2q, off, adam_t, t_off, cfg, dlogits, H, nf2, w2bf, f);
  else
    hipLaunchKernelGGL(fc1_conv_adam_fwd_kernel<64>, grid, dim3(256), 0, s, dH, a1, wslab1, wslab2, gb, B, params, m,
                       v, gdump, w1bf, w1tbf, w2r, w2q, off, adam_t, t_off, cfg, dlogits, H, nf2, w2bf, f);
}

void conv_adam(const float* wslab1, const float* wslab2, const float* gb, int B, float* params, float* m, float* v,
               float* gdump, uint16_t* w2r, uint16_t* w2q, Offsets off, const int* adam_t, int t_off, AdamCfg cfg,
               hipStream_t s) {
  hipLaunchKernelGGL(conv_adam_kernel, dim3(kC2 + kC1Blocks), dim3(256), 0, s, wslab1, wslab2, gb, B, params, m, v,
                     gdump, w2r, w2q, off, adam_t, t_off, cfg);
}

void init_fwd_attributes();

void init_attributes() {
  init_fwd_attributes();
  P2_CHECK(hipFuncSetAttribute(reinterpret_cast<const void*>(conv2_bwd_kernel),
                               hipFuncAttributeMaxDynamicSharedMemorySize, kDgLds));
  P2_CHECK(hipFuncSetAttribute(reinterpret_cast<const void*>(conv2_bwd_fc1_kernel<32>),
                               hipFuncAttributeMaxDynamicSharedMemorySize, kDgLds));
  P2_CHECK(hipFuncSetAttribute(reinterpret_cast<const void*>(conv2_bwd_fc1_kernel<64>),
                               hipFuncAttributeMaxDynamicSharedMemorySize, kDgLds));
  P2_CHECK(hipFuncSetAttribute(reinterpret_cast<const void*>(route_rm_kernel<1, 1>),
                               hipFuncAttributeMaxDynamicSharedMemorySize, kRouteRmLds));
  P2_CHECK(hipFuncSetAttribute(reinterpret_cast<const void*>(route_rm_kernel<2, 1>),
                               hipFuncAttributeMaxDynamicSharedMemorySize, kRouteRmLds));
  P2_CHECK(hipFuncSetAttribute(reinterpret_cast<const void*>(route_rm_kernel<1, 2>),
                               hipFuncAttributeMaxDynamicSharedMemorySize, kRouteRmLds / 2));
  P2_CHECK(hipFuncSetAttribute(reinterpret_cast<const void*>(route_rm_kernel<2, 2>),
                               hipFuncAttributeMaxDynamicSharedMemorySize, kRouteRmLds / 2));
}

}
```

### p2pfl_amd/learning/fused_cnn.py

```python

from __future__ import annotations

import collections
import math
import os
import threading
import time
from typing import Any, Dict, List, Optional, Tuple

import torch

from p2pfl_amd import ops
from p2pfl_amd.learning.arena import FlatParams, ModuleArena
from p2pfl_amd.learning.host_completion import HostCompletions
from p2pfl_amd.learning.torch_learner import TorchLearner
from p2pfl_amd.management.logger import logger
from p2pfl_amd.utils.lockcheck import make_lock, make_rlock
from p2pfl_amd.utils.streams import private_stream

_CAPTURE_LOCK = make_lock("FusedCNN._CAPTURE_LOCK")
RUN_AHEAD = max(1, int(os.environ.get("P2PFL_FIT_RUN_AHEAD", "2")))

_MERGED_ADAM = os.environ.get("P2PFL_CNN_MERGED_ADAM", "1") != "0"
_ROUTE_RM = os.environ.get("P2PFL_CNN_ROUTE_RM", "1") != "0"
_ROUTE_SPLIT = os.environ.get("P2PFL_CNN_ROUTE_SPLIT", "0") == "1"
_EVAL_LOW = os.environ.get("P2PFL_EVAL_STREAM_LOW", "1") != "0"
_EVAL_SIDE = os.environ.get("P2PFL_EVAL_SIDE_STREAM", "0")
_CONV12 = os.environ.get("P2PFL_CNN_CONV12", "0") == "1"
_FWD_IN_ADAM = os.environ.get("P2PFL_CNN_FWD_IN_ADAM", "0") == "1"
FC1_SLICE_DEFAULT = 384
FC1_TILES = 1600
_NAMES = ("conv1.weight", "conv1.bias", "conv2.weight", "conv2.bias", "l1.weight", "l1.bias", "l2.weight", "l2.bias")
FEAT, HID = 3136, 2048


class FusedCNNEngine:

    def __init__(
        self,
        model: torch.nn.Module,
        device: Optional[torch.device] = None,
        lr: float = 1e-3,
        betas: Tuple[float, float] = (0.9, 0.999),
        eps: float = 1e-8,
        weight_decay: float = 0.0,
        mrows: int = 32,
        arena: Optional[ModuleArena] = None,
        split_fc1: Optional[int] = None,
        fc1_slice: Optional[int] = None,
    ) -> None:
        self.C = ops.ext().cnn
        self.C.init()
        self.device = torch.device(device) if device is not None else torch.device("cuda", torch.cuda.current_device())
        model.to(self.device)
        self.arena = arena if arena is not None else ModuleArena(model, device=self.device)
        lay = self.arena.layout
        if tuple(lay.names) != _NAMES:
            raise ValueError(f"FusedCNNEngine needs the reference CNN layout {_NAMES}, got {lay.names}")
        shapes = dict(zip(lay.names, lay.shapes))
        if shapes["conv1.weight"] != (32, 1, 5, 5) or shapes["l2.weight"][1] != HID or shapes["l2.weight"][0] != 10:
            raise ValueError("unsupported CNN configuration (needs 1x28x28 input, 10 classes)")
        self.off: List[int] = [int(o) for o in lay.offsets]
        self.lr, self.betas, self.eps, self.wd = lr, betas, eps, weight_decay
        self.mrows = mrows
        self.S1 = int(split_fc1 if split_fc1 is not None else os.environ.get("P2PFL_CNN_FC1_SPLITS", "7"))
        if not 1 <= self.S1 <= 49:
            raise ValueError(f"FC1 split count {self.S1} outside [1, 49]")
        self.fc1_slice = int(fc1_slice if fc1_slice is not None else os.environ.get("P2PFL_CNN_FC1_SLICE", FC1_SLICE_DEFAULT))
        if not 0 <= self.fc1_slice <= FC1_TILES:
            raise ValueError(f"FC1 slice {self.fc1_slice} outside [0, {FC1_TILES}]")
        dev, bf = self.device, torch.bfloat16
        z = lambda *s, dt=torch.float32: torch.zeros(*s, dtype=dt, device=dev)
        n = self.arena.flat.numel()
        npad = (n + 3) // 4 * 4
        self._opt_state = z(2 * npad + 4)
        self.m, self.v = self._opt_state[:n], self._opt_state[npad:npad + n]
        self.adam_t = self._opt_state[2 * npad:2 * npad + 1].view(torch.int32)
        self.w2r, self.w2q = z(51200, dt=bf), z(51200, dt=bf)
        self.route_rm = _ROUTE_RM
        self.w1bf = z(HID * FEAT, dt=bf)
        self.w1tbf = None if self.route_rm else z(HID * FEAT, dt=bf)
        self.w2bf = z(10 * HID, dt=bf) if _MERGED_ADAM else None
        M = mrows
        self.p1, self.am1 = z(M * 196 * 32, dt=bf), z(M * 196 * 32, dt=torch.uint8)
        self.p1s = z(M * 5 * 32 * 18 * 16, dt=bf)
        self._a1s = (z(M * FEAT, dt=bf), z(M * FEAT, dt=bf))
        self._par = 0
        self.am2 = z(M * FEAT, dt=torch.uint8)
        self._fwd_sync = z(4, dt=torch.int32)
        self.slabs1 = z(self.S1 * M * HID)
        self.H, self.dH = z(M * HID, dt=bf), z(M * HID, dt=bf)
        self.dlogits = z(M * 10)
        self.dc2m, self.gb = z(M * 64 * 224, dt=bf), z(M * FEAT)
        self.wslab1, self.wslab2 = z(M * 7 * 832), z(self.C.wgrad_groups(M) * 51200)
        self.stats = z(2)
        split = self.route_rm and _ROUTE_SPLIT
        self.route_ws = z(98 * 2 * M * 32) if split else None
        self.route_ctr = z(98, dt=torch.int32) if split else None
        self.gdump: Optional[torch.Tensor] = None
        self.pack_shadows()

    @property
    def a1(self) -> torch.Tensor:
        return self._a1s[self._par]

    @property
    def params(self) -> torch.Tensor:
        return self.arena.flat

    @property
    def w1_route(self) -> torch.Tensor:
        return self.w1bf if self.route_rm else self.w1tbf

    def pack_shadows(self) -> None:
        self.C.pack_shadows(self.params, self.off, self.w2r, self.w2q, self.w1bf, self.w1tbf, self.w2bf)

    def reset_optimizer(self) -> None:
        self._opt_state.zero_()

    def _adam(self):
        return (self.lr, self.betas[0], self.betas[1], self.eps, self.wd)

    def forward(self, x: torch.Tensor, labels: torch.Tensor, idx: Optional[torch.Tensor], B: int, stats: torch.Tensor, train: bool,
                convs: bool = True) -> None:
        C, M = self.C, self.mrows
        if not convs:
            pass
        elif _CONV12:
            C.conv12_fwd(x, idx, self.params, self.off, self.w2r, None, self.am1, self.p1s if train else None, self.a1,
                         self.am2, B, M)
        else:
            C.conv1_fwd(x, idx, self.params, self.off, self.p1, self.am1, self.p1s if train else None, B)
            C.conv2_fwd(self.p1, self.w2r, self.params, self.off, self.a1, self.am2, B, M)
        C.gemm_skinny(self.a1, self.w1bf, self.slabs1, M, HID, FEAT, self.S1)
        C.head(self.slabs1, self.S1, M, self.params, self.off, labels, idx, B, train, self.H, self.dH, self.dlogits, stats,
               self.w2bf)

    def train_step_async(
        self, x: torch.Tensor, labels: torch.Tensor, idx: Optional[torch.Tensor], B: int, stats: torch.Tensor, t_off: int,
        nxt: Optional[Tuple[Optional[torch.Tensor], int]] = None, fwd_done: bool = False,
    ) -> None:
        if B > self.mrows:
            raise ValueError(f"batch {B} > engine capacity {self.mrows}")
        C, M, a = self.C, self.mrows, self._adam()
        self.forward(x, labels, idx, B, stats, True, convs=not fwd_done)
        if _MERGED_ADAM:
            C.route_fc2(self.dH, self.w1_route, self.am2, M, B, self.dc2m, self.gb, self.dlogits, self.H,
                        self.params, self.m, self.v, self.gdump, self.off, self.adam_t, t_off, *a, False, self.route_rm,
                        self.route_ws, self.route_ctr)
            if nxt is None and not fwd_done and self.fc1_slice:
                na = C.conv2_bwd_fc1(self.dc2m, self.p1s, self.am1, self.w2q, x, idx, self.wslab1, self.wslab2, B,
                                     self.dH, self.a1, M, self.params, self.m, self.v, self.gdump, self.w1bf,
                                     self.w1tbf, self.off, self.adam_t, t_off, *a, self.fc1_slice)
                C.fc1_conv_adam(self.dH, self.a1, M, self.wslab1, self.wslab2, self.gb, B, self.params, self.m, self.v,
                                self.gdump, self.w1bf, self.w1tbf, self.w2r, self.w2q, self.off, self.adam_t, t_off, *a,
                                self.dlogits, self.H, self.w2bf, na)
                return
            C.conv2_bwd(self.dc2m, self.p1s, self.am1, self.w2q, x, idx, self.wslab1, self.wslab2, B)
            if nxt is not None and M <= 64:
                idx_n, Bn = nxt
                C.fc1_conv_adam_fwd(self.dH, self.a1, M, self.wslab1, self.wslab2, self.gb, B, self.params, self.m,
                                    self.v, self.gdump, self.w1bf, self.w1tbf, self.w2r, self.w2q, self.off, self.adam_t,
                                    t_off, *a, self.dlogits, self.H, self.w2bf, x, idx_n, self.p1, self.am1, self.p1s,
                                    self._a1s[1 - self._par], self.am2, Bn, self._fwd_sync)
                self._par ^= 1
                return
            C.fc1_conv_adam(self.dH, self.a1, M, self.wslab1, self.wslab2, self.gb, B, self.params, self.m, self.v,
                            self.gdump, self.w1bf, self.w1tbf, self.w2r, self.w2q, self.off, self.adam_t, t_off, *a,
                            self.dlogits, self.H, self.w2bf)
            return
        C.route_fc2(self.dH, self.w1_route, self.am2, M, B, self.dc2m, self.gb, self.dlogits, self.H,
                    self.params, self.m, self.v, self.gdump, self.off, self.adam_t, t_off, *a, True, self.route_rm,
                    self.route_ws, self.route_ctr)
        C.fc1_wgrad_adam(self.dH, self.a1, M, self.params, self.m, self.v, self.gdump, self.w1bf, self.w1tbf, self.off, self.adam_t, t_off, *a)
        C.conv2_bwd(self.dc2m, self.p1s, self.am1, self.w2q, x, idx, self.wslab1, self.wslab2, B)
        C.conv_adam(self.wslab1, self.wslab2, self.gb, B, self.params, self.m, self.v, self.gdump, self.w2r, self.w2q, self.off, self.adam_t, t_off, *a)

    def train_step(self, x: torch.Tensor, y: torch.Tensor) -> float:
        B = int(y.shape[0])
        self.stats.zero_()
        self.train_step_async(x.contiguous(), y.to(torch.int64).contiguous(), None, B, self.stats, 1)
        self.adam_t += 1
        return float(self.stats[0]) / B

    @torch.no_grad()
    def logits_reference(self, x: torch.Tensor) -> torch.Tensor:
        return self.arena.module(x.float() / 255.0)


class _EvalSnapshot:

    READ = ("conv1.weight", "conv1.bias", "conv2.bias", "l1.bias", "l2.weight", "l2.bias")

    def __init__(self, eng: "FusedCNNEngine") -> None:
        self.params = torch.zeros_like(eng.params)
        self.w2r = torch.zeros_like(eng.w2r)
        self.w1bf = torch.zeros_like(eng.w1bf)
        self.w2bf = None if eng.w2bf is None else torch.zeros_like(eng.w2bf)
        ends = list(eng.off[1:]) + [eng.params.numel()]
        spans = sorted((eng.off[_NAMES.index(n)], ends[_NAMES.index(n)]) for n in self.READ)
        self.ranges: List[Tuple[int, int]] = []
        for a, b in spans:
            if self.ranges and self.ranges[-1][1] == a:
                self.ranges[-1] = (self.ranges[-1][0], b)
            else:
                self.ranges.append((a, b))
        self.done: Optional[torch.cuda.Event] = None

    def take(self, eng: "FusedCNNEngine") -> None:
        dst = [self.params[a:b] for a, b in self.ranges] + [self.w2r, self.w1bf]
        src = [eng.params[a:b] for a, b in self.ranges] + [eng.w2r, eng.w1bf]
        if self.w2bf is not None:
            dst.append(self.w2bf)
            src.append(eng.w2bf)
        ops.ext().fused.multi_copy(dst, src)


class _EvalForward:

    MROWS = 128

    def __init__(self, eng: FusedCNNEngine) -> None:
        self.eng = eng
        M, dev, bf = self.MROWS, eng.device, torch.bfloat16
        z = lambda *s, dt=torch.float32: torch.zeros(*s, dtype=dt, device=dev)
        self.p1, self.am1 = z(M * 196 * 32, dt=bf), z(M * 196 * 32, dt=torch.uint8)
        self.a1, self.am2 = z(M * FEAT, dt=bf), z(M * FEAT, dt=torch.uint8)
        self.slabs1 = z(eng.S1 * M * HID)
        self.H, self.dH = z(M * HID, dt=bf), z(M * HID, dt=bf)
        self.dlogits = z(M * 10)
        self.snaps: Dict[str, _EvalSnapshot] = {}

    def snapshot(self, name: str) -> _EvalSnapshot:
        if name not in self.snaps:
            self.snaps[name] = _EvalSnapshot(self.eng)
        return self.snaps[name]

    def forward(self, x: torch.Tensor, labels: torch.Tensor, idx: Optional[torch.Tensor], B: int, stats: torch.Tensor,
                snap: _EvalSnapshot) -> None:
        e, C, M = self.eng, self.eng.C, self.MROWS
        if _CONV12:
            C.conv12_fwd(x, idx, snap.params, e.off, snap.w2r, None, self.am1, None, self.a1, self.am2, B, M)
        else:
            C.conv1_fwd(x, idx, snap.params, e.off, self.p1, self.am1, None, B)
            C.conv2_fwd(self.p1, snap.w2r, snap.params, e.off, self.a1, self.am2, B, M)
        C.gemm_skinny(self.a1, snap.w1bf, self.slabs1, M, HID, FEAT, e.S1)
        C.head(self.slabs1, e.S1, M, snap.params, e.off, labels, idx, B, False, self.H, self.dH, self.dlogits, stats,
               snap.w2bf)


class _EpochGraph:

    def __init__(self, graph: Optional[torch.cuda.CUDAGraph], key: Tuple) -> None:
        self.graph = graph
        self.key = key


class FusedCNNLearner(TorchLearner):

    def __init__(self, model: Any, data: Any, self_addr: str, epochs: int, device: Optional[torch.device] = None, use_graphs: bool = True, **kw) -> None:
        super().__init__(model, data, self_addr, epochs, device=device, fused_optimizer=False)
        if self.device.type != "cuda":
            raise RuntimeError("FusedCNNLearner needs an AMD GPU")
        opt = model.configure_optimizers() if hasattr(model, "configure_optimizers") else None
        lr = float(opt.param_groups[0]["lr"]) if opt is not None else 1e-3
        betas = tuple(opt.param_groups[0].get("betas", (0.9, 0.999))) if opt is not None else (0.9, 0.999)
        eps = float(opt.param_groups[0].get("eps", 1e-8)) if opt is not None else 1e-8
        wd = float(opt.param_groups[0].get("weight_decay", 0.0)) if opt is not None else 0.0
        self.engine = FusedCNNEngine(model, self.device, lr=lr, betas=betas, eps=eps, weight_decay=wd, arena=self.arena)
        self.use_graphs = use_graphs
        self._graphs: Dict[str, _EpochGraph] = {}
        self._lock = make_rlock("FusedCNNLearner._lock")
        self._graph_build_lock = make_lock("FusedCNNLearner._graph_build_lock")
        self._stream = private_stream(self.device)
        self._dirty_shadows = False
        self._eval_fwd = _EvalForward(self.engine)
        self._completions = HostCompletions(self_addr)
        self._eval_stream = private_stream(self.device, 1 if _EVAL_LOW else 0)
        self._fit_hist: "collections.deque[torch.cuda.Event]" = collections.deque(maxlen=RUN_AHEAD)
        self._last_epoch_end: Optional[torch.cuda.Event] = None

    def set_parameters(self, params) -> None:
        if isinstance(params, FlatParams) and params.flat.data_ptr() == self.engine.params.data_ptr():
            self._arena_changed()
            return
        super().set_parameters(params)

    def _set_parameters(self, params) -> None:
        super()._set_parameters(params)
        self.engine.pack_shadows()

    def _plan(self, n: int, B: int) -> List[Tuple[int, int]]:
        return [(s, min(B, n - s)) for s in range(0, n, B)]

    def _graph_key(self, name: str, loader, train: bool):
        n = len(loader.dataset)
        B = loader.batch_size if train else _EvalForward.MROWS
        return self._plan(n, B), (name, n, B, loader.x.data_ptr(), loader.y.data_ptr())

    def _ensure_graph(self, name: str, loader, train: bool) -> "_EpochGraph":
        from p2pfl_amd.learning.step_graph import GATE

        plan, key = self._graph_key(name, loader, train)
        g = self._graphs.get(name)
        if g is not None and g.key == key:
            return g
        with self._graph_build_lock:
            g = self._graphs.get(name)
            if g is None or g.key != key:
                import gc

                with GATE.shared():
                    gc.collect()
                with GATE.exclusive():
                    g = self._capture(name, loader, plan, train, key)
                self._graphs[name] = g
        return g

    def _run(self, name: str, loader, train: bool, perm: Optional[torch.Tensor]) -> torch.Tensor:
        from p2pfl_amd.learning.step_graph import GATE

        plan, _ = self._graph_key(name, loader, train)
        g = self._ensure_graph(name, loader, train)
        with GATE.shared():
            if perm is not None:
                g.perm.copy_(perm, non_blocking=True)
            if g.graph is not None:
                g.graph.replay()
            else:
                g.stats.zero_()
                self._enqueue(name, loader, plan, train, g.perm, g.stats)
        return g.stats

    def _enqueue(self, name, loader, plan, train, perm, stats) -> None:
        x = loader.x.reshape(-1, 784)
        y = loader.y
        snap = None if train else self._eval_fwd.snapshot(name)
        chain = train and _FWD_IN_ADAM and _MERGED_ADAM and self.engine.mrows <= 64
        if train:
            self.engine._par = 0
        for j, (s, b) in enumerate(plan):
            idx = perm[s : s + b]
            st = stats[j] if train else stats[0]
            if train:
                nxt = None
                if chain and j + 1 < len(plan):
                    s2, b2 = plan[j + 1]
                    nxt = (perm[s2 : s2 + b2], b2)
                self.engine.train_step_async(x, y, idx, b, st, j + 1, nxt=nxt, fwd_done=chain and j > 0)
            else:
                self._eval_fwd.forward(x, y, idx, b, st, snap)

    def _capture(self, name, loader, plan, train, key) -> _EpochGraph:
        n = len(loader.dataset)
        if not train:
            self._eval_fwd.snapshot(name)
        eg = _EpochGraph(None, key)
        eg.perm = torch.arange(n, dtype=torch.int64, device=self.device)
        eg.stats = torch.zeros((len(plan) if train else 1, 4), dtype=torch.float32, device=self.device)
        if not self.use_graphs:
            return eg
        from p2pfl_amd.learning.step_graph import no_gc

        with _CAPTURE_LOCK:
            torch.cuda.synchronize(self.device)
            graph = torch.cuda.CUDAGraph()
            with no_gc(collect=False), torch.cuda.graph(graph, stream=self._stream, capture_error_mode="relaxed"):
                eg.stats.zero_()
                self._enqueue(name, loader, plan, train, eg.perm, eg.stats)
            torch.cuda.synchronize(self.device)
        eg.graph = graph
        return eg

    @staticmethod
    def _readback(stats: torch.Tensor) -> torch.Tensor:
        from p2pfl_amd.learning.step_graph import GATE

        with GATE.shared():
            host = torch.empty(stats.shape, dtype=stats.dtype, pin_memory=True)
            host.copy_(stats, non_blocking=True)
        return host

    def fit(self) -> None:
        if self.epochs <= 0 or self.model is None:
            return
        try:
            with self._on_stream():
                self._fit_fused()
        finally:
            self._arena_changed()

    def _fit_fused(self) -> None:
        from p2pfl_amd.learning.step_graph import GATE

        self._interrupt.clear()
        self._arena_changed()
        if len(self._fit_hist) == RUN_AHEAD:
            self._fit_hist[0].synchronize()
        self._ensure_graph("train", self.data.train_dataloader(), True)
        val = self.data.val_dataloader()
        if val is not None and len(val.dataset) > 0:
            self._ensure_graph("val", val, False)
        with self._lock:
            self.engine.reset_optimizer()
            loader = self.data.train_dataloader()
            n, bs = len(loader.dataset), loader.batch_size
            steps = math.ceil(n / bs)
            cur = torch.cuda.current_stream(self.device)
            for epoch in range(self.epochs):
                if self._interrupt.is_set():
                    return
                if epoch:
                    self.engine.adam_t.fill_(epoch * steps)
                t0, t1 = torch.cuda.Event(enable_timing=True), torch.cuda.Event(enable_timing=True)
                t0.record(cur)
                with GATE.shared():
                    perm = loader.permutation(host=True)
                stats = self._run("train", loader, True, perm)
                t1.record(cur)
                host = self._readback(stats)
                done = torch.cuda.Event()
                done.record(cur)
                base = self._step
                self._step += steps
                prev, self._last_epoch_end = self._last_epoch_end, t1
                self._completions.submit(done, lambda h=host, b=base, a=t0, z=t1, p=prev: self._log_epoch(h, b, steps, bs, n, a, z, p))
                self._validate_async()
            fit_done = torch.cuda.Event()
            fit_done.record(cur)
            self._fit_hist.append(fit_done)

    def _log_epoch(self, host: torch.Tensor, base: int, steps: int, bs: int, n: int, t0: Any, t1: Any, prev_end: Any = None) -> None:
        loss_sums = [row[0] for row in host.tolist()]
        every = max(1, self.log_every_n_steps)
        for j in range(steps):
            if (base + j + 1) % every == 0:
                self._log("train_loss", loss_sums[j] / min(bs, n - j * bs), step=base + j + 1)
        self.last_train_loss = sum(loss_sums) / n
        ms = t0.elapsed_time(t1)
        logger.tracer.record(self._addr, "train_epoch_gpu", time.perf_counter() - ms * 1e-3, ms * 1e-3)
        if prev_end is not None:
            gap = prev_end.elapsed_time(t0)
            logger.tracer.record(self._addr, "inter_epoch_gpu", time.perf_counter() - gap * 1e-3, gap * 1e-3)

    def _eval_async(self, name: str, loader, on_done) -> None:
        self._ensure_graph(name, loader, False)
        snap = self._eval_fwd.snapshot(name)
        cur = torch.cuda.current_stream(self.device)
        side = self._stream_for_block() is not None if _EVAL_SIDE == "auto" else _EVAL_SIDE != "0"
        es = self._eval_stream if side else cur
        with self._lock:
            if snap.done is not None:
                cur.wait_event(snap.done)
            snap.take(self.engine)
            es.wait_stream(cur)
            with torch.cuda.stream(es):
                stats = self._run(name, loader, False, None)
                host = self._readback(stats[0, :2])
                ev = torch.cuda.Event()
                ev.record(es)
            snap.done = ev
        n = max(1, len(loader.dataset))

        def fin() -> None:
            loss, correct = host.tolist()
            on_done(loss / n, correct / n)

        self._completions.submit(ev, fin)
        return ev

    def _validate_async(self) -> None:
        loader = self.data.val_dataloader()
        if loader is None or len(loader.dataset) == 0:
            return
        step = self._step
        self._eval_async("val", loader, lambda loss, acc: (self._log("val_loss", loss, step=step), self._log("val_metric", acc, step=step)))

    def _validate(self) -> None:
        self._validate_async()
        self._completions.drain()

    def evaluate_async(self, on_results: Optional[Any] = None) -> bool:
        if self.epochs <= 0 or self.model is None:
            return False

        def done(loss: float, acc: float) -> None:
            results = {"test_loss": loss, "test_metric": acc}
            for k, v in results.items():
                self._log(k, v)
            if on_results is not None:
                on_results(results)

        with logger.span(self._addr, "evaluate"), self._on_stream(writes=False):
            self._eval_async("test", self.data.test_dataloader(), done)
        return True

    def evaluate(self) -> Dict[str, float]:
        box: Dict[str, float] = {}
        if not self.evaluate_async(box.update):
            return {}
        self._completions.drain()
        return box

    def drain(self, timeout: Optional[float] = None) -> bool:
        return self._completions.drain(timeout)


def auto_learner(model: Any, data: Any, self_addr: str, epochs: int, **kw):
    from p2pfl_amd.models.cnn import CNN

    if isinstance(model, CNN) and torch.cuda.is_available() and ops.available():
        return FusedCNNLearner(model, data, self_addr, epochs, **kw)
    return TorchLearner(model, data, self_addr, epochs, **kw)
```

Before: 423,600 samples/s.

## Double-buffer W1 bf16 shadow so routing launch can host FC1 Adam tiles

Adds a second bf16 W1 shadow buffer that alternates each step, so the row-major dA1 routing kernel can read the current W1 while FC1 weight-gradient and Adam tiles, now hosted inside the routing launch, write the next copy. The FC1 tiles are spread across the routing, conv2-backward and fused Adam launches using a first_tile offset. This fills idle blocks in the routing launch and shortens the serial tail. FC1 param, m and v streams also gain a nontemporal load/store option. The cost is an extra 12.8MB buffer and a copy to settle the shadow when an odd step count leaves the pointer flipped, which is skipped during graph capture.

```diff
diff --git a/csrc/cnn.h b/csrc/cnn.h
--- a/csrc/cnn.h
+++ b/csrc/cnn.h
@@ -62,7 +62,8 @@
   float* m;
   float* v;
   float* gdump;
-  uint16_t* w1bf;
+  const uint16_t* w1bf;
+  uint16_t* w1bf_w;
   uint16_t* w1tbf;
   Offsets off;
   const int* adam_t;
@@ -72,7 +73,12 @@
 
 int conv2_bwd_fc1(const uint16_t* dc2m, const uint16_t* p1s, const uint8_t* am1, const uint16_t* w2q, const uint8_t* x,
                   const int64_t* idx, float* wslab1, float* wslab2, int B, const Fc1Args& f, int n_tiles,
-                  hipStream_t s);
+                  int first_tile, hipStream_t s);
+
+int route_rm_fc1(const uint16_t* dH, const uint16_t* w1, const uint8_t* am2, int mrows, int B, uint16_t* dc2m,
+                 float* gb, const float* dlogits, const uint16_t* H, float* params, float* m, float* v, float* gdump,
+                 Offsets off, const int* adam_t, int t_off, AdamCfg cfg, bool with_fc2, const Fc1Args& f, int n_tiles,
+                 hipStream_t s);
 
 void conv_adam(const float* wslab1, const float* wslab2, const float* gb, int B, float* params, float* m, float* v,
                float* gdump, uint16_t* w2r, uint16_t* w2q, Offsets off, const int* adam_t, int t_off, AdamCfg cfg,
diff --git a/csrc/cnn_bindings.cpp b/csrc/cnn_bindings.cpp
--- a/csrc/cnn_bindings.cpp
+++ b/csrc/cnn_bindings.cpp
@@ -179,9 +179,55 @@
   }
 }
 
+p2cnn::Fc1Args fc1_args(const torch::Tensor& dH, const torch::Tensor& a1, int64_t mrows, const torch::Tensor& params,
+                        const torch::Tensor& m, const torch::Tensor& v, const c10::optional<torch::Tensor>& gdump,
+                        const torch::Tensor& w1bf_w, const c10::optional<torch::Tensor>& w1tbf, const Offsets& o,
+                        const torch::Tensor& adam_t, int64_t t_off, const AdamCfg& c) {
+  const int64_t n = params_end(o);
+  p2cnn::Fc1Args fc{};
+  fc.dH = reinterpret_cast<uint16_t*>(ptr<at::BFloat16>(dH, torch::kBFloat16, mrows * 2048, "dH"));
+  fc.a1 = reinterpret_cast<uint16_t*>(ptr<at::BFloat16>(a1, torch::kBFloat16, mrows * 3136, "a1"));
+  fc.mrows = int(mrows);
+  fc.params = ptr<float>(params, torch::kFloat32, n, "params");
+  fc.m = ptr<float>(m, torch::kFloat32, n, "m");
+  fc.v = ptr<float>(v, torch::kFloat32, n, "v");
+  fc.gdump = optr<float>(gdump, torch::kFloat32, n, "gdump");
+  fc.w1bf_w = reinterpret_cast<uint16_t*>(ptr<at::BFloat16>(w1bf_w, torch::kBFloat16, 2048 * 3136, "w1bf"));
+  fc.w1tbf = reinterpret_cast<uint16_t*>(optr<at::BFloat16>(w1tbf, torch::kBFloat16, 2048 * 3136, "w1tbf"));
+  fc.off = o;
+  fc.adam_t = ptr<int>(adam_t, torch::kInt32, 1, "adam_t", 4);
+  fc.t_off = int(t_off);
+  fc.cfg = c;
+  return fc;
+}
+
+int64_t k_route_rm_fc1(torch::Tensor dH, torch::Tensor w1, torch::Tensor am2, int64_t mrows, int64_t B,
+                       torch::Tensor dc2m, torch::Tensor gb, torch::Tensor dlogits, torch::Tensor H, torch::Tensor params,
+                       torch::Tensor m, torch::Tensor v, c10::optional<torch::Tensor> gdump, std::vector<int64_t> off,
+                       torch::Tensor adam_t, int64_t t_off, double lr, double b1, double b2, double eps, double wd,
+                       bool with_fc2, torch::Tensor a1, torch::Tensor w1_write, int64_t n_tiles) {
+  const c10::DeviceGuard g(dH.device());
+  check_batch(int(B), int(mrows));
+  TORCH_CHECK(mrows <= 64, "route_rm_fc1: mrows must be 32 or 64");
+  TORCH_CHECK(n_tiles >= 0 && n_tiles <= p2cnn::kFc1Tiles, "route_rm_fc1: n_tiles ", n_tiles, " outside [0, ",
+              p2cnn::kFc1Tiles, "]");
+  Offsets o = offsets(off);
+  p2cnn::Fc1Args fc = fc1_args(dH, a1, mrows, params, m, v, gdump, w1_write, c10::nullopt, o, adam_t, t_off,
+                               cfg(lr, b1, b2, eps, wd));
+  fc.w1bf = reinterpret_cast<uint16_t*>(ptr<at::BFloat16>(w1, torch::kBFloat16, 2048 * 3136, "w1"));
+  TORCH_CHECK(n_tiles == 0 || fc.w1bf != fc.w1bf_w,
+              "route_rm_fc1: hosted FC1 tiles must write the other W1 shadow buffer than the routing blocks read");
+  return p2cnn::route_rm_fc1(
+      fc.dH, fc.w1bf, ptr<uint8_t>(am2, torch::kUInt8, B * 3136, "am2"), int(mrows), int(B),
+      reinterpret_cast<uint16_t*>(ptr<at::BFloat16>(dc2m, torch::kBFloat16, B * 64 * 224, "dc2m")),
+      ptr<float>(gb, torch::kFloat32, B * 3136, "gb"), ptr<float>(dlogits, torch::kFloat32, B * 10, "dlogits"),
+      reinterpret_cast<uint16_t*>(ptr<at::BFloat16>(H, torch::kBFloat16, B * 2048, "H")), fc.params, fc.m, fc.v,
+      fc.gdump, o, fc.adam_t, int(t_off), fc.cfg, with_fc2, fc, int(n_tiles), stream());
+}
+
 int64_t conv2_bwd_impl(torch::Tensor dc2m, torch::Tensor p1s, torch::Tensor am1, torch::Tensor w2q, torch::Tensor x,
                        c10::optional<torch::Tensor> idx, torch::Tensor wslab1, torch::Tensor wslab2, int64_t B,
-                       const p2cnn::Fc1Args& fc, int64_t n_tiles) {
+                       const p2cnn::Fc1Args& fc, int64_t n_tiles, int64_t first_tile) {
   TORCH_CHECK(B >= 1 && B <= 64, "bad batch");
   TORCH_CHECK(x.numel() % 784 == 0, "x must be [N,1,28,28] uint8");
   if (!idx.has_value()) TORCH_CHECK(x.numel() / 784 >= B, "x has fewer than B rows");
@@ -193,13 +239,13 @@
       ptr<uint8_t>(x, torch::kUInt8, 784, "x", 1), idx_ptr(idx, B),
       ptr<float>(wslab1, torch::kFloat32, B * p2cnn::kDgTiles * p2cnn::kSlab1, "wslab1"),
       ptr<float>(wslab2, torch::kFloat32, p2cnn::wgrad_groups(int(B)) * int64_t(p2cnn::kSlab2), "wslab2"), int(B), fc,
-      int(n_tiles), stream());
+      int(n_tiles), int(first_tile), stream());
 }
 
 void k_conv2_bwd(torch::Tensor dc2m, torch::Tensor p1s, torch::Tensor am1, torch::Tensor w2q, torch::Tensor x,
                  c10::optional<torch::Tensor> idx, torch::Tensor wslab1, torch::Tensor wslab2, int64_t B) {
   const c10::DeviceGuard g(dc2m.device());
-  conv2_bwd_impl(dc2m, p1s, am1, w2q, x, idx, wslab1, wslab2, B, p2cnn::Fc1Args{}, 0);
+  conv2_bwd_impl(dc2m, p1s, am1, w2q, x, idx, wslab1, wslab2, B, p2cnn::Fc1Args{}, 0, 0);
 }
 
 int64_t k_conv2_bwd_fc1(torch::Tensor dc2m, torch::Tensor p1s, torch::Tensor am1, torch::Tensor w2q, torch::Tensor x,
@@ -207,28 +253,18 @@
                         torch::Tensor dH, torch::Tensor a1, int64_t mrows, torch::Tensor params, torch::Tensor m,
                         torch::Tensor v, c10::optional<torch::Tensor> gdump, torch::Tensor w1bf,
                         c10::optional<torch::Tensor> w1tbf, std::vector<int64_t> off, torch::Tensor adam_t,
-                        int64_t t_off, double lr, double b1, double b2, double eps, double wd, int64_t n_tiles) {
+                        int64_t t_off, double lr, double b1, double b2, double eps, double wd, int64_t n_tiles,
+                        int64_t first_tile) {
   const c10::DeviceGuard g(dc2m.device());
   TORCH_CHECK(mrows == 32 || mrows == 64, "conv2_bwd_fc1: mrows must be 32 or 64");
   TORCH_CHECK(n_tiles >= 0 && n_tiles <= p2cnn::kFc1Tiles, "conv2_bwd_fc1: n_tiles ", n_tiles, " outside [0, ",
               p2cnn::kFc1Tiles, "]");
-  Offsets o = offsets(off);
-  const int64_t n = params_end(o);
-  p2cnn::Fc1Args fc{};
-  fc.dH = reinterpret_cast<uint16_t*>(ptr<at::BFloat16>(dH, torch::kBFloat16, mrows * 2048, "dH"));
-  fc.a1 = reinterpret_cast<uint16_t*>(ptr<at::BFloat16>(a1, torch::kBFloat16, mrows * 3136, "a1"));
-  fc.mrows = int(mrows);
-  fc.params = ptr<float>(params, torch::kFloat32, n, "params");
-  fc.m = ptr<float>(m, torch::kFloat32, n, "m");
-  fc.v = ptr<float>(v, torch::kFloat32, n, "v");
-  fc.gdump = optr<float>(gdump, torch::kFloat32, n, "gdump");
-  fc.w1bf = reinterpret_cast<uint16_t*>(ptr<at::BFloat16>(w1bf, torch::kBFloat16, 2048 * 3136, "w1bf"));
-  fc.w1tbf = reinterpret_cast<uint16_t*>(optr<at::BFloat16>(w1tbf, torch::kBFloat16, 2048 * 3136, "w1tbf"));
-  fc.off = o;
-  fc.adam_t = ptr<int>(adam_t, torch::kInt32, 1, "adam_t", 4);
-  fc.t_off = int(t_off);
-  fc.cfg = cfg(lr, b1, b2, eps, wd);
-  return conv2_bwd_impl(dc2m, p1s, am1, w2q, x, idx, wslab1, wslab2, B, fc, n_tiles);
+  TORCH_CHECK(first_tile >= 0 && first_tile + n_tiles <= p2cnn::kFc1Tiles, "conv2_bwd_fc1: first_tile ", first_tile,
+              " + n_tiles ", n_tiles, " outside [0, ", p2cnn::kFc1Tiles, "]");
+  Offsets o = offsets(off);
+  const p2cnn::Fc1Args fc =
+      fc1_args(dH, a1, mrows, params, m, v, gdump, w1bf, w1tbf, o, adam_t, t_off, cfg(lr, b1, b2, eps, wd));
+  return conv2_bwd_impl(dc2m, p1s, am1, w2q, x, idx, wslab1, wslab2, B, fc, n_tiles, first_tile);
 }
 
 void k_conv_adam(torch::Tensor wslab1, torch::Tensor wslab2, torch::Tensor gb, int64_t B, torch::Tensor params,
@@ -367,8 +403,15 @@
         pybind11::arg("ws") = pybind11::none(), pybind11::arg("ctr") = pybind11::none());
   c.def("fc1_wgrad_adam", &k_fc1_wgrad_adam);
   c.def("conv2_bwd", &k_conv2_bwd);
-  c.def("conv2_bwd_fc1", &k_conv2_bwd_fc1,
-        "conv2_bwd hosting the first n_tiles FC1 weight-gradient + Adam tiles; returns the tiles hosted");
+  namespace py = pybind11;
+  c.def("route_rm_fc1", &k_route_rm_fc1,
+        "the row-major dA1 routing launch hosting FC1 tiles [0, n_tiles), which write w1_write; returns the tiles hosted");
+  c.def("conv2_bwd_fc1", &k_conv2_bwd_fc1, py::arg("dc2m"), py::arg("p1s"), py::arg("am1"), py::arg("w2q"), py::arg("x"),
+        py::arg("idx"), py::arg("wslab1"), py::arg("wslab2"), py::arg("B"), py::arg("dH"), py::arg("a1"), py::arg("mrows"),
+        py::arg("params"), py::arg("m"), py::arg("v"), py::arg("gdump"), py::arg("w1bf"), py::arg("w1tbf"), py::arg("off"),
+        py::arg("adam_t"), py::arg("t_off"), py::arg("lr"), py::arg("b1"), py::arg("b2"), py::arg("eps"), py::arg("wd"),
+        py::arg("n_tiles"), py::arg("first_tile") = 0,
+        "conv2_bwd hosting n_tiles FC1 weight-gradient + Adam tiles from first_tile on; returns the tiles hosted");
   c.def("conv_adam", &k_conv_adam);
   c.def("fc1_conv_adam", &k_fc1_conv_adam, pybind11::arg("dH"), pybind11::arg("a1"), pybind11::arg("mrows"), pybind11::arg("wslab1"),
         pybind11::arg("wslab2"), pybind11::arg("gb"), pybind11::arg("B"), pybind11::arg("params"), pybind11::arg("m"), pybind11::arg("v"), pybind11::arg("gdump"),
diff --git a/csrc/cnn_bwd.hip b/csrc/cnn_bwd.hip
--- a/csrc/cnn_bwd.hip
+++ b/csrc/cnn_bwd.hip
@@ -185,16 +185,13 @@
 }
 
 template <int MT, int KS>
-__global__ __launch_bounds__(512) void route_rm_kernel(const uint16_t* __restrict__ dH,
-                                                       const uint16_t* __restrict__ w1,
-                                                       const uint8_t* __restrict__ am2, int B,
-                                                       uint16_t* __restrict__ dc2m, float* __restrict__ gb,
-                                                       const float* __restrict__ dlogits,
-                                                       const uint16_t* __restrict__ H, float* __restrict__ p,
-                                                       float* __restrict__ m, float* __restrict__ v,
-                                                       float* __restrict__ gdump, Offsets off,
-                                                       const int* __restrict__ adam_t, int t_off, AdamCfg cfg,
-                                                       float* __restrict__ ws, int* __restrict__ ctr, int xa) {
+P2_DEVICE void route_rm_block(const uint16_t* __restrict__ dH, const uint16_t* __restrict__ w1,
+                              const uint8_t* __restrict__ am2, int B, uint16_t* __restrict__ dc2m,
+                              float* __restrict__ gb, const float* __restrict__ dlogits,
+                              const uint16_t* __restrict__ H, float* __restrict__ p, float* __restrict__ m,
+                              float* __restrict__ v, float* __restrict__ gdump, const Offsets& off,
+                              const int* __restrict__ adam_t, int t_off, const AdamCfg& cfg,
+                              float* __restrict__ ws, int* __restrict__ ctr, int xa) {
   constexpr int NB = kRouteBlocks * KS;
   const int nbl = xa ? 8 * xa : NB;
   if (int(blockIdx.x) >= nbl) {
@@ -329,6 +326,20 @@
     *reinterpret_cast<uint32_t*>(row) = top;
     *reinterpret_cast<uint32_t*>(row + 16) = bot;
   }
+}
+
+template <int MT, int KS>
+__global__ __launch_bounds__(512) void route_rm_kernel(const uint16_t* __restrict__ dH,
+                                                       const uint16_t* __restrict__ w1,
+                                                       const uint8_t* __restrict__ am2, int B,
+                                                       uint16_t* __restrict__ dc2m, float* __restrict__ gb,
+                                                       const float* __restrict__ dlogits,
+                                                       const uint16_t* __restrict__ H, float* __restrict__ p,
+                                                       float* __restrict__ m, float* __restrict__ v,
+                                                       float* __restrict__ gdump, Offsets off,
+                                                       const int* __restrict__ adam_t, int t_off, AdamCfg cfg,
+                                                       float* __restrict__ ws, int* __restrict__ ctr, int xa) {
+  route_rm_block<MT, KS>(dH, w1, am2, B, dc2m, gb, dlogits, H, p, m, v, gdump, off, adam_t, t_off, cfg, ws, ctr, xa);
 }
 
 void route_fc2_rm(const uint16_t* dH, const uint16_t* w1, const uint8_t* am2, int mrows, int B, uint16_t* dc2m,
@@ -373,19 +384,40 @@
   static constexpr int kBytes = kMain + 128 * 40 * 2;
 };
 
-template <int MR>
+typedef float f32x4v __attribute__((ext_vector_type(4)));
+template <bool NT>
+P2_DEVICE float4 fc1_ld4(const float* q) {
+  if constexpr (NT) {
+    const f32x4v t = __builtin_nontemporal_load(reinterpret_cast<const f32x4v*>(q));
+    return make_float4(t.x, t.y, t.z, t.w);
+  } else {
+    return *reinterpret_cast<const float4*>(q);
+  }
+}
+template <bool NT>
+P2_DEVICE void fc1_st4(float* q, const float4& u) {
+  if constexpr (NT) {
+    f32x4v t = {u.x, u.y, u.z, u.w};
+    __builtin_nontemporal_store(t, reinterpret_cast<f32x4v*>(q));
+  } else {
+    *reinterpret_cast<float4*>(q) = u;
+  }
+}
+
+template <int MR, bool NT = false>
 P2_DEVICE void fc1_wgrad_adam_body(int bx, int by, const uint16_t* __restrict__ dH, const uint16_t* __restrict__ a1,
                                    float* __restrict__ p, float* __restrict__ m, float* __restrict__ v,
                                    float* __restrict__ gdump, uint16_t* __restrict__ w1bf,
                                    uint16_t* __restrict__ w1tbf, const Offsets& off,
-                                   const int* __restrict__ adam_t, int t_off, const AdamCfg& cfg, char* smem) {
+                                   const int* __restrict__ adam_t, int t_off, const AdamCfg& cfg, char* smem,
+                                   int tid) {
   constexpr int AP = Fc1Lds<MR>::AP;
   constexpr int GP = Fc1Lds<MR>::GP;
   uint16_t(*tr)[40] = reinterpret_cast<uint16_t(*)[40]>(smem + Fc1Lds<MR>::kMain);
   uint16_t* sdh = reinterpret_cast<uint16_t*>(smem);
   uint16_t* sa1 = sdh + MR * 32;
   float(*gt)[GP] = reinterpret_cast<float(*)[GP]>(smem);
-  const int tid = threadIdx.x, wave = tid >> 6, lane = tid & 63, r = lane & 31, h = lane >> 5;
+  const int wave = tid >> 6, lane = tid & 63, r = lane & 31, h = lane >> 5;
   const int n0 = by * 32;
   const int kb = bx * 128;
   const int nl = tid >> 3, kq = (tid & 7) * 4;
@@ -398,9 +430,9 @@
     const int k = kb + kq + 32 * j;
     if (k < kFeat) {
       const int64_t e = int64_t(n0 + nl) * kFeat + k;
-      pr[j] = *reinterpret_cast<const float4*>(pw + e);
-      mr[j] = *reinterpret_cast<const float4*>(mw + e);
-      vr[j] = *reinterpret_cast<const float4*>(vw + e);
+      pr[j] = fc1_ld4<NT>(pw + e);
+      mr[j] = fc1_ld4<NT>(mw + e);
+      vr[j] = fc1_ld4<NT>(vw + e);
     }
   }
   for (int i = tid; i < MR * 4; i += 256) {
@@ -458,9 +490,9 @@
     adam_regs(pr[j].y, mr[j].y, vr[j].y, g.y, cfg, s);
     adam_regs(pr[j].z, mr[j].z, vr[j].z, g.z, cfg, s);
     adam_regs(pr[j].w, mr[j].w, vr[j].w, g.w, cfg, s);
-    *reinterpret_cast<float4*>(pw + e) = pr[j];
-    *reinterpret_cast<float4*>(mw + e) = mr[j];
-    *reinterpret_cast<float4*>(vw + e) = vr[j];
+    fc1_st4<NT>(pw + e, pr[j]);
+    fc1_st4<NT>(mw + e, mr[j]);
+    fc1_st4<NT>(vw + e, vr[j]);
     const uint16_t b0 = f32_to_bf16(pr[j].x), b1 = f32_to_bf16(pr[j].y), b2 = f32_to_bf16(pr[j].z),
                    b3 = f32_to_bf16(pr[j].w);
     uint2 o;
@@ -491,7 +523,7 @@
                                                              Offsets off, const int* __restrict__ adam_t, int t_off,
                                                              AdamCfg cfg) {
   __shared__ __attribute__((aligned(16))) char smem[Fc1Lds<MR>::kBytes];
-  fc1_wgrad_adam_body<MR>(blockIdx.x, blockIdx.y, dH, a1, p, m, v, gdump, w1bf, w1tbf, off, adam_t, t_off, cfg, smem);
+  fc1_wgrad_adam_body<MR>(blockIdx.x, blockIdx.y, dH, a1, p, m, v, gdump, w1bf, w1tbf, off, adam_t, t_off, cfg, smem, threadIdx.x);
 }
 
 void fc1_wgrad_adam(const uint16_t* dH, const uint16_t* a1, int mrows, float* params, float* m, float* v,
@@ -504,6 +536,50 @@
   else
     hipLaunchKernelGGL(fc1_wgrad_adam_kernel<64>, grid, dim3(256), 0, s, dH, a1, params, m, v, gdump, w1bf, w1tbf,
                        off, adam_t, t_off, cfg);
+}
+
+template <int MT>
+__global__ __launch_bounds__(512) void route_rm_fc1_kernel(
+    const uint16_t* __restrict__ dH, const uint16_t* __restrict__ w1, const uint8_t* __restrict__ am2, int B,
+    uint16_t* __restrict__ dc2m, float* __restrict__ gb, const float* __restrict__ dlogits,
+    const uint16_t* __restrict__ H, float* __restrict__ p, float* __restrict__ m, float* __restrict__ v,
+    float* __restrict__ gdump, Offsets off, const int* __restrict__ adam_t, int t_off, AdamCfg cfg, int xa, int nroute,
+    Fc1Args f, int n_fc1) {
+  static_assert(2 * Fc1Lds<32 * MT>::kBytes <= kRouteRmLds, "two FC1 tiles fit the launch's dynamic LDS");
+  if (int(blockIdx.x) < nroute) {
+    route_rm_block<MT, 1>(dH, w1, am2, B, dc2m, gb, dlogits, H, p, m, v, gdump, off, adam_t, t_off, cfg, nullptr,
+                          nullptr, xa);
+    return;
+  }
+  extern __shared__ __attribute__((aligned(16))) char smem[];
+  constexpr int kBx = (kFeat + 127) / 128;
+  const int half = threadIdx.x >> 8;
+  const int t = 2 * (int(blockIdx.x) - nroute) + half;
+  if (t >= n_fc1) return;
+  fc1_wgrad_adam_body<32 * MT, true>(t % kBx, t / kBx, f.dH, f.a1, f.params, f.m, f.v, f.gdump, f.w1bf_w, f.w1tbf,
+                                     f.off, f.adam_t, f.t_off, f.cfg, smem + half * (kRouteRmLds / 2),
+                                     threadIdx.x & 255);
+}
+
+int route_rm_fc1(const uint16_t* dH, const uint16_t* w1, const uint8_t* am2, int mrows, int B, uint16_t* dc2m,
+                 float* gb, const float* dlogits, const uint16_t* H, float* params, float* m, float* v, float* gdump,
+                 Offsets off, const int* adam_t, int t_off, AdamCfg cfg, bool with_fc2, const Fc1Args& f, int n_tiles,
+                 hipStream_t s) {
+  if (n_tiles == 0) {
+    route_fc2_rm(dH, w1, am2, mrows, B, dc2m, gb, dlogits, H, params, m, v, gdump, off, adam_t, t_off, cfg, with_fc2,
+                 nullptr, nullptr, s);
+    return 0;
+  }
+  const int xa = xcd_align() ? kRouteBlocks / kXcdSplits : 0;
+  const int nroute = (xa ? 8 * xa : kRouteBlocks) + (with_fc2 ? kFc2Blocks : 0);
+  const dim3 grid(nroute + (n_tiles + 1) / 2);
+  if (mrows == 32)
+    hipLaunchKernelGGL(route_rm_fc1_kernel<1>, grid, dim3(512), kRouteRmLds, s, dH, w1, am2, B, dc2m, gb, dlogits, H,
+                       params, m, v, gdump, off, adam_t, t_off, cfg, xa, nroute, f, n_tiles);
+  else
+    hipLaunchKernelGGL(route_rm_fc1_kernel<2>, grid, dim3(512), kRouteRmLds, s, dH, w1, am2, B, dc2m, gb, dlogits, H,
+                       params, m, v, gdump, off, adam_t, t_off, cfg, xa, nroute, f, n_tiles);
+  return n_tiles;
 }
 
 constexpr int kOCP = 72;
@@ -801,7 +877,7 @@
     const uint16_t* __restrict__ dc2m, const uint16_t* __restrict__ p1s, const uint8_t* __restrict__ am1,
     const uint16_t* __restrict__ w2q, const uint8_t* __restrict__ xds, const int64_t* __restrict__ idx,
     float* __restrict__ wslab1, float* __restrict__ wslab2, int B, int nconv, int wg_blocks, int stream_w,
-    int wg_first, Fc1Args f) {
+    int wg_first, Fc1Args f, int f0) {
   static_assert(Fc1Lds<MR>::kBytes <= kDgLds, "the launch's dynamic LDS serves the FC1 role too");
   extern __shared__ __attribute__((aligned(16))) char smem[];
   constexpr int kBx = (kFeat + 127) / 128;
@@ -810,14 +886,14 @@
     conv2_bwd_roles(j, nconv, dc2m, p1s, am1, w2q, xds, idx, wslab1, wslab2, B, wg_blocks, stream_w, wg_first, smem);
     return;
   }
-  const int t = j - nconv;
-  fc1_wgrad_adam_body<MR>(t % kBx, t / kBx, f.dH, f.a1, f.params, f.m, f.v, f.gdump, f.w1bf, f.w1tbf, f.off, f.adam_t,
-                          f.t_off, f.cfg, smem);
+  const int t = j - nconv + f0;
+  fc1_wgrad_adam_body<MR>(t % kBx, t / kBx, f.dH, f.a1, f.params, f.m, f.v, f.gdump, f.w1bf_w, f.w1tbf, f.off, f.adam_t,
+                          f.t_off, f.cfg, smem, threadIdx.x);
 }
 
 int conv2_bwd_fc1(const uint16_t* dc2m, const uint16_t* p1s, const uint8_t* am1, const uint16_t* w2q, const uint8_t* x,
                   const int64_t* idx, float* wslab1, float* wslab2, int B, const Fc1Args& f, int n_tiles,
-                  hipStream_t s) {
+                  int first_tile, hipStream_t s) {
   static const int roles = [] {
     const char* e = getenv("P2CNN_CONV2BWD_ROLES");
     return e ? atoi(e) : 3;
@@ -843,16 +919,16 @@
                        wslab2, B, first, wg_blocks, stream_w, roles == 3 ? wg_first : 0);
   else if (f.mrows == 32)
     hipLaunchKernelGGL(conv2_bwd_fc1_kernel<32>, dim3(blocks + na), dim3(256), kDgLds, s, dc2m, p1s, am1, w2q, x, idx,
-                       wslab1, wslab2, B, blocks, wg_blocks, stream_w, wg_first, f);
+                       wslab1, wslab2, B, blocks, wg_blocks, stream_w, wg_first, f, first_tile);
   else
     hipLaunchKernelGGL(conv2_bwd_fc1_kernel<64>, dim3(blocks + na), dim3(256), kDgLds, s, dc2m, p1s, am1, w2q, x, idx,
-                       wslab1, wslab2, B, blocks, wg_blocks, stream_w, wg_first, f);
+                       wslab1, wslab2, B, blocks, wg_blocks, stream_w, wg_first, f, first_tile);
   return na;
 }
 
 void conv2_bwd(const uint16_t* dc2m, const uint16_t* p1s, const uint8_t* am1, const uint16_t* w2q, const uint8_t* x,
                const int64_t* idx, float* wslab1, float* wslab2, int B, hipStream_t s) {
-  conv2_bwd_fc1(dc2m, p1s, am1, w2q, x, idx, wslab1, wslab2, B, Fc1Args{}, 0, s);
+  conv2_bwd_fc1(dc2m, p1s, am1, w2q, x, idx, wslab1, wslab2, B, Fc1Args{}, 0, 0, s);
 }
 
 constexpr int kC1Blocks = kSlab1 / 16;
@@ -1031,7 +1107,7 @@
     return;
   }
   const int f = j - kCA + f0;
-  fc1_wgrad_adam_body<MR>(f % kBx, f / kBx, dH, a1, p, m, v, gdump, w1bf, w1tbf, off, adam_t, t_off, cfg, smem);
+  fc1_wgrad_adam_body<MR>(f % kBx, f / kBx, dH, a1, p, m, v, gdump, w1bf, w1tbf, off, adam_t, t_off, cfg, smem, threadIdx.x);
 }
 
 void fc1_conv_adam(const uint16_t* dH, const uint16_t* a1, int mrows, const float* wslab1, const float* wslab2,
@@ -1095,7 +1171,7 @@
   j -= kCA;
   constexpr int nfc1 = kBx * (kHid / 32);
   if (j < nfc1) {
-    fc1_wgrad_adam_body<MR>(j % kBx, j / kBx, dH, a1, p, m, v, gdump, w1bf, w1tbf, off, adam_t, t_off, cfg, smem);
+    fc1_wgrad_adam_body<MR>(j % kBx, j / kBx, dH, a1, p, m, v, gdump, w1bf, w1tbf, off, adam_t, t_off, cfg, smem, threadIdx.x);
     return;
   }
   j -= nfc1;
@@ -1164,6 +1240,10 @@
                                hipFuncAttributeMaxDynamicSharedMemorySize, kRouteRmLds / 2));
   P2_CHECK(hipFuncSetAttribute(reinterpret_cast<const void*>(route_rm_kernel<2, 2>),
                                hipFuncAttributeMaxDynamicSharedMemorySize, kRouteRmLds / 2));
-}
-
-}
+  P2_CHECK(hipFuncSetAttribute(reinterpret_cast<const void*>(route_rm_fc1_kernel<1>),
+                               hipFuncAttributeMaxDynamicSharedMemorySize, kRouteRmLds));
+  P2_CHECK(hipFuncSetAttribute(reinterpret_cast<const void*>(route_rm_fc1_kernel<2>),
+                               hipFuncAttributeMaxDynamicSharedMemorySize, kRouteRmLds));
+}
+
+}
diff --git a/p2pfl_amd/learning/fused_cnn.py b/p2pfl_amd/learning/fused_cnn.py
--- a/p2pfl_amd/learning/fused_cnn.py
+++ b/p2pfl_amd/learning/fused_cnn.py
@@ -28,8 +28,9 @@
 _EVAL_SIDE = os.environ.get("P2PFL_EVAL_SIDE_STREAM", "0")
 _CONV12 = os.environ.get("P2PFL_CNN_CONV12", "0") == "1"
 _FWD_IN_ADAM = os.environ.get("P2PFL_CNN_FWD_IN_ADAM", "0") == "1"
-FC1_SLICE_DEFAULT = 384
+FC1_SLICE_DEFAULT = 448
 FC1_TILES = 1600
+ROUTE_SLICE_DEFAULT = 288
 _NAMES = ("conv1.weight", "conv1.bias", "conv2.weight", "conv2.bias", "l1.weight", "l1.bias", "l2.weight", "l2.bias")
 FEAT, HID = 3136, 2048
 
@@ -48,6 +49,7 @@
         arena: Optional[ModuleArena] = None,
         split_fc1: Optional[int] = None,
         fc1_slice: Optional[int] = None,
+        route_slice: Optional[int] = None,
     ) -> None:
         self.C = ops.ext().cnn
         self.C.init()
@@ -69,6 +71,11 @@
         self.fc1_slice = int(fc1_slice if fc1_slice is not None else os.environ.get("P2PFL_CNN_FC1_SLICE", FC1_SLICE_DEFAULT))
         if not 0 <= self.fc1_slice <= FC1_TILES:
             raise ValueError(f"FC1 slice {self.fc1_slice} outside [0, {FC1_TILES}]")
+        room = FC1_TILES - self.fc1_slice
+        rs = route_slice if route_slice is not None else os.environ.get("P2PFL_CNN_ROUTE_SLICE")
+        self.route_slice = int(rs) if rs is not None else min(ROUTE_SLICE_DEFAULT, room)
+        if not 0 <= self.route_slice <= room:
+            raise ValueError(f"route slice {self.route_slice} outside [0, {room}] (1600 - fc1_slice)")
         dev, bf = self.device, torch.bfloat16
         z = lambda *s, dt=torch.float32: torch.zeros(*s, dtype=dt, device=dev)
         n = self.arena.flat.numel()
@@ -79,6 +86,9 @@
         self.w2r, self.w2q = z(51200, dt=bf), z(51200, dt=bf)
         self.route_rm = _ROUTE_RM
         self.w1bf = z(HID * FEAT, dt=bf)
+        self._hop_arm = _MERGED_ADAM and self.route_rm and not _ROUTE_SPLIT and not _FWD_IN_ADAM
+        self._w1s = (self.w1bf, z(HID * FEAT, dt=bf) if self._hop_arm else None)
+        self._wp = 0
         self.w1tbf = None if self.route_rm else z(HID * FEAT, dt=bf)
         self.w2bf = z(10 * HID, dt=bf) if _MERGED_ADAM else None
         M = mrows
@@ -109,8 +119,21 @@
         return self.arena.flat
 
     @property
+    def w1_cur(self) -> torch.Tensor:
+        return self._w1s[self._wp]
+
+    @property
     def w1_route(self) -> torch.Tensor:
-        return self.w1bf if self.route_rm else self.w1tbf
+        return self.w1_cur if self.route_rm else self.w1tbf
+
+    def hop_steps(self, steps: int) -> int:
+        return steps - steps % 2 if self._hop_arm and self.route_slice else 0
+
+    def settle_shadow(self) -> None:
+        if self._wp:
+            if not torch.cuda.is_current_stream_capturing():
+                self.w1bf.copy_(self._w1s[1])
+            self._wp = 0
 
     def pack_shadows(self) -> None:
         self.C.pack_shadows(self.params, self.off, self.w2r, self.w2q, self.w1bf, self.w1tbf, self.w2bf)
@@ -132,47 +155,62 @@
         else:
             C.conv1_fwd(x, idx, self.params, self.off, self.p1, self.am1, self.p1s if train else None, B)
             C.conv2_fwd(self.p1, self.w2r, self.params, self.off, self.a1, self.am2, B, M)
-        C.gemm_skinny(self.a1, self.w1bf, self.slabs1, M, HID, FEAT, self.S1)
+        C.gemm_skinny(self.a1, self.w1_cur, self.slabs1, M, HID, FEAT, self.S1)
         C.head(self.slabs1, self.S1, M, self.params, self.off, labels, idx, B, train, self.H, self.dH, self.dlogits, stats,
                self.w2bf)
 
     def train_step_async(
         self, x: torch.Tensor, labels: torch.Tensor, idx: Optional[torch.Tensor], B: int, stats: torch.Tensor, t_off: int,
-        nxt: Optional[Tuple[Optional[torch.Tensor], int]] = None, fwd_done: bool = False,
+        nxt: Optional[Tuple[Optional[torch.Tensor], int]] = None, fwd_done: bool = False, hop: bool = False,
     ) -> None:
         if B > self.mrows:
             raise ValueError(f"batch {B} > engine capacity {self.mrows}")
+        if hop and not (self._hop_arm and nxt is None and not fwd_done):
+            raise ValueError("only the default step can hop between the W1 shadow buffers")
         C, M, a = self.C, self.mrows, self._adam()
         self.forward(x, labels, idx, B, stats, True, convs=not fwd_done)
+        if hop:
+            w1r, w1w = self.w1_cur, self._w1s[1 - self._wp]
+            nr = C.route_rm_fc1(self.dH, w1r, self.am2, M, B, self.dc2m, self.gb, self.dlogits, self.H, self.params,
+                                self.m, self.v, self.gdump, self.off, self.adam_t, t_off, *a, False, self.a1, w1w,
+                                self.route_slice)
+            na = nr + C.conv2_bwd_fc1(self.dc2m, self.p1s, self.am1, self.w2q, x, idx, self.wslab1, self.wslab2, B,
+                                      self.dH, self.a1, M, self.params, self.m, self.v, self.gdump, w1w, None,
+                                      self.off, self.adam_t, t_off, *a, self.fc1_slice, nr)
+            C.fc1_conv_adam(self.dH, self.a1, M, self.wslab1, self.wslab2, self.gb, B, self.params, self.m, self.v,
+                            self.gdump, w1w, None, self.w2r, self.w2q, self.off, self.adam_t, t_off, *a,
+                            self.dlogits, self.H, self.w2bf, na)
+            self._wp ^= 1
+            return
         if _MERGED_ADAM:
             C.route_fc2(self.dH, self.w1_route, self.am2, M, B, self.dc2m, self.gb, self.dlogits, self.H,
                         self.params, self.m, self.v, self.gdump, self.off, self.adam_t, t_off, *a, False, self.route_rm,
                         self.route_ws, self.route_ctr)
             if nxt is None and not fwd_done and self.fc1_slice:
                 na = C.conv2_bwd_fc1(self.dc2m, self.p1s, self.am1, self.w2q, x, idx, self.wslab1, self.wslab2, B,
-                                     self.dH, self.a1, M, self.params, self.m, self.v, self.gdump, self.w1bf,
+                                     self.dH, self.a1, M, self.params, self.m, self.v, self.gdump, self.w1_cur,
                                      self.w1tbf, self.off, self.adam_t, t_off, *a, self.fc1_slice)
                 C.fc1_conv_adam(self.dH, self.a1, M, self.wslab1, self.wslab2, self.gb, B, self.params, self.m, self.v,
-                                self.gdump, self.w1bf, self.w1tbf, self.w2r, self.w2q, self.off, self.adam_t, t_off, *a,
+                                self.gdump, self.w1_cur, self.w1tbf, self.w2r, self.w2q, self.off, self.adam_t, t_off, *a,
                                 self.dlogits, self.H, self.w2bf, na)
                 return
             C.conv2_bwd(self.dc2m, self.p1s, self.am1, self.w2q, x, idx, self.wslab1, self.wslab2, B)
             if nxt is not None and M <= 64:
                 idx_n, Bn = nxt
                 C.fc1_conv_adam_fwd(self.dH, self.a1, M, self.wslab1, self.wslab2, self.gb, B, self.params, self.m,
-                                    self.v, self.gdump, self.w1bf, self.w1tbf, self.w2r, self.w2q, self.off, self.adam_t,
+                                    self.v, self.gdump, self.w1_cur, self.w1tbf, self.w2r, self.w2q, self.off, self.adam_t,
                                     t_off, *a, self.dlogits, self.H, self.w2bf, x, idx_n, self.p1, self.am1, self.p1s,
                                     self._a1s[1 - self._par], self.am2, Bn, self._fwd_sync)
                 self._par ^= 1
                 return
             C.fc1_conv_adam(self.dH, self.a1, M, self.wslab1, self.wslab2, self.gb, B, self.params, self.m, self.v,
-                            self.gdump, self.w1bf, self.w1tbf, self.w2r, self.w2q, self.off, self.adam_t, t_off, *a,
+                            self.gdump, self.w1_cur, self.w1tbf, self.w2r, self.w2q, self.off, self.adam_t, t_off, *a,
                             self.dlogits, self.H, self.w2bf)
             return
         C.route_fc2(self.dH, self.w1_route, self.am2, M, B, self.dc2m, self.gb, self.dlogits, self.H,
                     self.params, self.m, self.v, self.gdump, self.off, self.adam_t, t_off, *a, True, self.route_rm,
                     self.route_ws, self.route_ctr)
-        C.fc1_wgrad_adam(self.dH, self.a1, M, self.params, self.m, self.v, self.gdump, self.w1bf, self.w1tbf, self.off, self.adam_t, t_off, *a)
+        C.fc1_wgrad_adam(self.dH, self.a1, M, self.params, self.m, self.v, self.gdump, self.w1_cur, self.w1tbf, self.off, self.adam_t, t_off, *a)
         C.conv2_bwd(self.dc2m, self.p1s, self.am1, self.w2q, x, idx, self.wslab1, self.wslab2, B)
         C.conv_adam(self.wslab1, self.wslab2, self.gb, B, self.params, self.m, self.v, self.gdump, self.w2r, self.w2q, self.off, self.adam_t, t_off, *a)
 
@@ -339,17 +377,21 @@
         chain = train and _FWD_IN_ADAM and _MERGED_ADAM and self.engine.mrows <= 64
         if train:
             self.engine._par = 0
-        for j, (s, b) in enumerate(plan):
-            idx = perm[s : s + b]
-            st = stats[j] if train else stats[0]
-            if train:
-                nxt = None
-                if chain and j + 1 < len(plan):
-                    s2, b2 = plan[j + 1]
-                    nxt = (perm[s2 : s2 + b2], b2)
-                self.engine.train_step_async(x, y, idx, b, st, j + 1, nxt=nxt, fwd_done=chain and j > 0)
-            else:
-                self._eval_fwd.forward(x, y, idx, b, st, snap)
+        hops = self.engine.hop_steps(len(plan)) if train else 0
+        try:
+            for j, (s, b) in enumerate(plan):
+                idx = perm[s : s + b]
+                st = stats[j] if train else stats[0]
+                if train:
+                    nxt = None
+                    if chain and j + 1 < len(plan):
+                        s2, b2 = plan[j + 1]
+                        nxt = (perm[s2 : s2 + b2], b2)
+                    self.engine.train_step_async(x, y, idx, b, st, j + 1, nxt=nxt, fwd_done=chain and j > 0, hop=j < hops)
+                else:
+                    self._eval_fwd.forward(x, y, idx, b, st, snap)
+        finally:
+            self.engine.settle_shadow()
 
     def _capture(self, name, loader, plan, train, key) -> _EpochGraph:
         n = len(loader.dataset)
```

Result: faster. 437,400 samples/s, median of 6 (+3.3%).
